# retinal-information-processing-lab/gaussian_processes

Hardware: AMD Instinct MI355X
Metric: GP fits/sec (kernel+chol+solve+grad loglik) at N=8192 d=256 (higher is better)
Workload: dtype f64; 1 GPU; N=8192 d=256 single cell f64, one M-step closure evaluation with 6 gradients (BASELINE configs[2], headline); N=8192, d=256, parallelism=independent units over 1 GPU(s), one process per GPU, no data-path collective

## Files before the change

### gaussian_processes_amd/_lib.py

```python
from __future__ import annotations

import ctypes
import os

from .build import lib_path

vp, i32, i64, f64 = ctypes.c_void_p, ctypes.c_int, ctypes.c_int64, ctypes.c_double
pd = ctypes.POINTER(ctypes.c_double)



class DevGemmArgs(ctypes.Structure):
    _fields_ = ([(n, vp) for n in ("A", "B", "C")] + [(n, i64) for n in ("lda", "ldb", "ldc", "sA", "sB", "sC")] +
                [("alpha", f64), ("beta", f64)] +
                [(n, vp) for n in ("sk_ws", "aux", "sumsq", "Ap", "Bp", "Cp", "auxp", "sumsqp")] +
                [(n, ctypes.c_int32) for n in ("M", "N", "K", "a_kmajor", "b_kmajor", "out_lower", "a_tri", "b_tri", "batch",
                                               "split_k", "tile", "walk", "epi", "nptr", "k_slabs", "b_split")])


class DevGemmRoute(ctypes.Structure):
    _fields_ = [(n, ctypes.c_int32) for n in ("rc", "tile", "sk_first", "xcd", "stages", "half_occ", "edge", "epi",
                                              "sumsq_entries", "blocks", "pair", "slabs")]


_SIGS = {
    "gpfit_version": (i32, []),
    "gpfit_last_error": (ctypes.c_char_p, []),
    "gpfit_dgemm": (i32, [vp, i32, i32, i32, i32, i32, f64, vp, i64, vp, i64, f64, vp, i64, i32, i32, i32]),
    "gpfit_dgemm_ex": (i32, [vp, i32, i32, i32, i32, i32, f64, vp, i64, vp, i64, f64, vp, i64, i32, i32, i32, i32, i32]),
    "gpfit_ctx_create": (i32, [i32, i64, i64, i64, ctypes.POINTER(vp)]),
    "gpfit_ctx_destroy": (None, [vp]),
    "gpfit_check_limits": (i32, [pd, pd, pd]),
    "gpfit_localker_mask": (i32, [pd, i32, i32, vp, ctypes.POINTER(i64)]),
    "gpfit_localker": (i32, [vp, vp, pd, i32, i32, vp, i64, vp, vp]),
    "gpfit_acosker": (i32, [vp, vp, f64, vp, i64, i64, vp, i64, i64, i64, vp, i64, vp, vp, i64, vp]),
    "gpfit_acosker_pullback": (i32, [vp, vp, f64, vp, i64, i64, vp, i64, i64, i64, vp, i64, vp, i64, vp, vp, i64, pd]),
    "gpfit_acosker_diag": (i32, [vp, vp, f64, vp, i64, i64, i64, vp, i64, vp, vp, vp]),
    "gpfit_fit_eval": (i32, [vp, vp, pd, pd, pd, i32, i32, vp, i64, i64, vp, vp, vp, i64, f64, f64, i32, pd,
                             vp, vp, vp]),
    "gpfit_potrf": (i32, [vp, vp, vp, i64, i64, vp, i64, vp, i64, pd, ctypes.POINTER(i32)]),
    "gpfit_potrf_append": (i32, [vp, vp, vp, i64, vp, i64, i64, vp, pd, ctypes.POINTER(i32)]),
    "gpfit_potrf_append_block": (i32, [vp, vp, vp, i64, vp, i64, i64, i64, vp, i64, pd, ctypes.POINTER(i32)]),
    "gpfit_estep": (i32, [vp, vp, vp, i64, i64, vp, vp, vp, f64, vp, vp, i64]),
    "gpfit_estep_projected": (i32, [vp, vp, vp, i64, vp, i64, vp, i64, i64, i64, vp, vp, vp, f64, vp, vp, i64, vp, vp,
                                    vp]),
    "gpfit_estep_projected_damped": (i32, [vp, vp, vp, i64, vp, i64, vp, i64, vp, i64, vp, i64, i64, i64, vp, vp, vp, f64, f64,
                                           vp, vp, i64, ctypes.POINTER(i32)]),
    "gpfit_fparam_eval": (i32, [vp, vp, vp, vp, vp, i64, f64, i32, f64, vp, pd]),
    "gpfit_fparam_lbfgs": (i32, [vp, vp, vp, vp, vp, i64, f64, i32, f64, i32, i32, f64, f64, f64, vp, pd]),
    "gpfit_estep_chain": (i32, [vp, vp, vp, i64, vp, i64, vp, i64, i64, i64, vp, vp, vp, vp, vp, i64, vp, vp, f64, i32, f64,
                                i32, i32, i32, f64, f64, f64, pd]),
    "gpfit_estep_chain_full": (i32, [vp, vp, vp, i64, i64, vp, vp, vp, vp, vp, i64, vp, vp, f64, i32, f64, i32, i32, i32, f64,
                                     f64, f64, pd]),
    "gpfit_estep_chain_batch": (i32, [vp, i32, vp, vp, vp, vp, vp, vp, vp, i64, vp, vp, vp, vp, vp, vp, vp, vp, vp, pd, i32, pd,
                                      i32, i32, i32, f64, f64, f64, pd]),
    "gpfit_estep_chain_full_batch": (i32, [vp, i32, vp, vp, vp, i64, vp, vp, vp, vp, vp, vp, vp, vp, pd, i32, pd, i32, i32, i32,
                                           f64, f64, f64, pd]),
    "gpfit_estep_chain_damped": (i32, [vp, vp, vp, i64, vp, i64, vp, i64, vp, i64, i64, i64, vp, vp, vp, vp, vp, i64, vp, vp,
                                       f64, f64, i32, f64, i32, i32, i32, f64, f64, f64, pd]),
    "gpfit_estep_chain_damped_batch": (i32, [vp, i32, vp, vp, vp, vp, vp, vp, vp, vp, vp, i64, vp, vp, vp, vp, vp, vp, vp, vp,
                                             vp, pd, f64, i32, pd, i32, i32, i32, f64, f64, f64, pd]),
    "gpfit_elbo": (i32, [vp, vp, vp, vp, i64, vp, i64, vp, i64, i64, i32, f64, vp, vp, vp, i64, f64, f64, pd,
                         ctypes.POINTER(i32)]),
    "gpfit_elbo_batch": (i32, [vp, i32, vp, vp, vp, vp, vp, vp, vp, vp, vp, ctypes.POINTER(i32), pd, vp, vp, vp, i64, pd, pd, pd,
                               ctypes.POINTER(i32)]),
    "gpfit_subspace_sweeps": (i32, [vp, vp, vp, i64, i64, i64, vp, vp, vp, vp, i32, pd, i32, ctypes.POINTER(i32)]),
    "gpfit_subspace_sweeps_batch": (i32, [vp, i32, vp, vp, i64, i64, i64, vp, vp, vp, vp, ctypes.POINTER(i32), vp, i32,
                                          ctypes.POINTER(i32)]),
    "gpfit_sign_steps": (i32, [vp, vp, vp, i64, f64, vp, vp, vp, i32, pd, i32, i32, ctypes.POINTER(i32)]),
    "gpfit_sign_steps_batch": (i32, [vp, i32, vp, vp, i64, pd, vp, vp, vp, i32, pd, i32, i32, ctypes.POINTER(i32)]),
    "gpfit_fparam_lbfgs_host": (i32, [vp, vp, vp, i64, f64, i32, f64, i32, i32, f64, f64, f64, vp, pd]),
    "gpfit_set_profile": (i32, [vp, i32]),
    "gpfit_get_profile": (i32, [vp, pd]),
    "gpfit_get_phases": (i32, [vp, pd]),
    "gpfit_last_enqueue_ms": (f64, [vp]),
    "gpfit_fit_eval_f32": (i32, [vp, vp, pd, pd, pd, i32, i32, vp, i64, i64, vp, vp, vp, i64, f64, f64, i32, pd,
                                 vp, vp, vp]),
    "gpfit_fit_eval_finish": (i32, [vp, pd]),
    "gpfit_fit_eval_batch": (i32, [vp, i32, vp, pd, pd, pd, i32, i32, vp, i64, i64, vp, vp, vp, i64, pd, pd, i32, pd,
                                   ctypes.POINTER(i32)]),
    "gpfit_fit_eval_batch_f32": (i32, [vp, i32, vp, pd, pd, pd, i32, i32, vp, i64, i64, vp, vp, vp, i64, pd, pd, i32, pd,
                                       ctypes.POINTER(i32)]),
    "gpfit_fit_eval_projected": (i32, [vp, vp, pd, pd, pd, i32, i32, vp, i64, i64, vp, vp, i64, i64, vp, vp, i64, f64, f64, pd]),
    "gpfit_fit_eval_projected_batch": (i32, [vp, i32, vp, pd, pd, pd, i32, i32, vp, i64, i64, vp, vp, vp, vp, vp, vp, vp, pd, pd,
                                             pd, ctypes.POINTER(i32)]),
    "gpfit_fit_eval_sparse": (i32, [vp, vp, pd, pd, pd, i32, i32, vp, i64, i64, vp, i64, i64, vp, vp, i64, i64, vp, vp, i64,
                                    f64, f64, pd]),
    "gpfit_fit_eval_sparse_batch": (i32, [vp, i32, vp, pd, pd, pd, i32, i32, vp, i64, i64, vp, i64, i64, vp, vp, vp, vp, vp,
                                          vp, vp, pd, pd, pd, ctypes.POINTER(i32)]),
    "gpfit_grad_pullback": (i32, [vp, vp, pd, i32, i32, vp, i64, i64, vp, i64, vp, pd]),
    "gpfit_nd_utility": (i32, [vp, vp, vp, i64, vp, i32, vp]),
    "gpfit_score_pool": (i32, [vp, vp, f64, vp, i64, i64, vp, i64, vp, i64, i64, i64, vp, i64, vp, i64, i64, vp, i64, vp,
                               f64, f64, vp, i32, i64, vp, vp, vp, vp]),
    "gpfit_score_pool_batch": (i32, [vp, i32, vp, pd, vp, vp, i64, vp, vp, vp, vp, vp, vp, vp, vp, vp, vp, vp, vp, vp, vp, pd, pd,
                                     vp, i32, i64, vp, vp, vp, vp]),
    "gpfit_utility_sum": (i32, [vp, vp, i64, i32, vp, i64, vp]),
    "gpfit_probe_mfma_f64": (i32, [vp, vp, i32, i32]),
    "gpfit_probe_stream_copy": (i32, [vp, vp, vp, i64]),
    "gpfit_dev_gemm_route": (i32, [i32, ctypes.POINTER(DevGemmArgs), ctypes.POINTER(DevGemmArgs), ctypes.POINTER(DevGemmRoute)]),
    "gpfit_dev_gemm_plan": (i64, [i32, ctypes.POINTER(DevGemmArgs), i32, ctypes.POINTER(ctypes.c_int32), i64]),
    "gpfit_dev_gemm": (i32, [vp, i32, ctypes.POINTER(DevGemmArgs), ctypes.POINTER(DevGemmArgs)]),
    "gpfit_dev_ctx_copy": (i32, [vp, ctypes.c_char_p, i64, vp, i64, i32]),
    "gpfit_dev_ctx_fill": (i32, [vp, ctypes.c_char_p, i32]),
    "gpfit_dev_potrf": (i32, [vp, vp, i32, i32, vp, vp, vp, vp, vp, i64, i32, ctypes.c_uint32, ctypes.c_uint32, i32]),
}

_lib = None


class GpfitError(RuntimeError):
    pass


def exported_symbols():
    return sorted(_SIGS)


def load():
    global _lib
    if _lib is not None:
        return _lib
    path = lib_path()
    if not os.path.exists(path):
        raise GpfitError(
            f"{path} not found: build it with `python -m gaussian_processes_amd.build` "
            "(there is no CPU fallback for the GP fit path)")
    lib = ctypes.CDLL(path)
    for name, (res, args) in _SIGS.items():
        fn = getattr(lib, name)
        fn.restype = res
        fn.argtypes = args
    _lib = lib
    return lib


def last_error() -> str:
    return load().gpfit_last_error().decode(errors="replace")


def check(rc: int, what: str):
    if rc < 0 and rc != -2:
        raise GpfitError(f"{what} failed (rc={rc}): {last_error()}")
    return rc


def darr(values):
    return (ctypes.c_double * len(values))(*[float(v) for v in values])
```

### gaussian_processes_amd/csrc/api_dev.hip

```cpp
#include "gemm_core.h"
#include "context.h"
#include "gpfit_mi355x.h"

#include <cstring>

namespace gpfit {
namespace {

template <typename R>
int fill(const gpfit_dev_gemm_args& d, GemmArgsT<R>& g) {
  g = GemmArgsT<R>{};
  g.A = (const R*)d.A; g.B = (const R*)d.B; g.C = (R*)d.C;
  g.lda = d.lda; g.ldb = d.ldb; g.ldc = d.ldc;
  g.M = d.M; g.N = d.N; g.K = d.K;
  g.alpha = d.alpha; g.beta = d.beta;
  g.a_kmajor = d.a_kmajor; g.b_kmajor = d.b_kmajor;
  g.out_lower = d.out_lower; g.a_tri = d.a_tri; g.b_tri = d.b_tri;
  g.batch = d.batch > 0 ? d.batch : 1;
  g.sA = d.sA; g.sB = d.sB; g.sC = d.sC;
  g.split_k = d.split_k > 0 ? d.split_k : 1;
  g.k_slabs = d.k_slabs > 0 ? d.k_slabs : 0;
  g.tile = d.tile;
  g.reverse = d.walk & 15;
  g.half_occ = (d.walk >> 4) & 1;
  g.sk_ws = d.sk_ws;
  g.epi = d.epi;
  g.aux = (R*)d.aux;
  g.sumsq = d.sumsq;
  g.b_split = d.b_split;
  g.nptr = d.nptr;
  if (d.nptr < 0 || d.nptr > GEMM_MAXB) return d.nptr < 0 ? -3 : 0;
  for (int b = 0; b < d.nptr; ++b) {
    if (!d.Ap || !d.Bp || !d.Cp) return -3;
    g.Ap[b] = (const R*)d.Ap[b];
    g.Bp[b] = (const R*)d.Bp[b];
    g.Cp[b] = (R*)d.Cp[b];
    g.auxp[b] = d.auxp ? (R*)d.auxp[b] : nullptr;
    g.sumsqp[b] = d.sumsqp ? d.sumsqp[b] : nullptr;
  }
  return 0;
}

template <typename R>
int route(const gpfit_dev_gemm_args& d, const gpfit_dev_gemm_args* d2, gpfit_dev_gemm_route_t& o) {
  std::memset(&o, 0, sizeof(o));
  o.sk_first = -1;
  GemmArgsT<R> a, b;
  if (fill(d, a) != 0 || (d2 && fill(*d2, b) != 0)) return -3;
  GemmRoute r = d2 ? gemm_pair_shape(a, b) : gemm_route(a);
  long blocks = d2 ? r.tiles : -1;
  if (r.rc == 0 && r.sched == GEMM_STREAMK) {
    SkHostPlan plan;
    if (streamk_plan_host(a, r.sk_first, plan) != 0) r.stay_data_parallel();
    else blocks = plan.blocks;
  }
  if (r.rc == 0 && r.sched == GEMM_XCD) {
    std::vector<int> table;
    if (xcd_plan_host(a, table) != 0) return -3;
    r.gx = (int)table.size();
  }
  o.rc = r.rc; o.tile = r.tile; o.sk_first = r.sk_first; o.xcd = r.sched == GEMM_XCD; o.stages = r.stages;
  o.half_occ = r.half; o.edge = r.edge; o.epi = r.epi; o.sumsq_entries = r.sumsq_entries; o.slabs = r.slabs;
  o.pair = d2 && r.rc == 0;
  o.blocks = (int)std::min<long>(blocks >= 0 ? blocks : (long)r.gx * r.gy * r.gz, 0x7fffffffL);
  return 0;
}

template <typename R>
int64_t plan(const gpfit_dev_gemm_args& d, int kind, int32_t* out, int64_t cap) {
  GemmArgsT<R> a;
  if (fill(d, a) != 0 || a.M <= 0 || a.N <= 0) return -3;
  const GemmRoute r = gemm_route(a);
  if (r.rc != 0) return -3;
  if (kind == 1) {
    if (r.sched != GEMM_XCD) return -1;
    std::vector<int> table;
    if (xcd_plan_host(a, table) != 0) return -1;
    const int64_t need = 1 + (int64_t)table.size();
    if (need > cap || !out) return need;
    out[0] = (int32_t)table.size();
    std::memcpy(out + 1, table.data(), table.size() * sizeof(int));
    return need;
  }
  if (kind == 4) {
    if (r.sched != GEMM_XCD) return -1;
    std::vector<int> table;
    if (xcd_plan_host(a, table) != 0) return -1;
    const int64_t need = 1 + 3 * (int64_t)table.size();
    if (need > cap || !out) return need;
    out[0] = (int32_t)table.size();
    for (size_t e = 0; e < table.size(); ++e) {
      const int t = table[e];
      KRange kr{0, 0};
      if (t >= 0) kr = gemm_tile_k_range(a.a_tri, a.b_tri, a.K, (t >> 16) * TILE, (t & 0xffff) * TILE, TILE, a.b_split);
      out[1 + 3 * e] = t; out[2 + 3 * e] = kr.beg; out[3 + 3 * e] = kr.end;
    }
    return need;
  }
  if (kind == 3) {
    if (a.k_slabs <= 0) return -1;
    const SlabPlan sp = slab_plan(a.M, a.k_slabs);
    const int64_t need = 4 + 4 * (int64_t)sp.items;
    if (need > cap || !out) return need;
    out[0] = sp.items; out[1] = sp.live; out[2] = sp.ks * SLAB_TILE; out[3] = SLAB_TILE;
    for (int e = 0; e < sp.items; ++e) {
      int ti, z;
      slab_item(sp, e, ti, z);
      int32_t* w = out + 4 + 4 * e;
      w[0] = ti; w[1] = z;
      const KRange kr = gemm_tile_k_range(a.a_tri, a.b_tri, a.K, ti * SLAB_TILE, 0, SLAB_TILE);
      w[2] = std::max(kr.beg, z * sp.ks * SLAB_TILE);
      w[3] = std::min(kr.end, (z + 1) * sp.ks * SLAB_TILE);
    }
    return need;
  }
  if (kind != 2) return -3;
  if (r.sched != GEMM_STREAMK) return -1;
  const int first = r.sk_first;
  SkHostPlan p;
  if (streamk_plan_host(a, first, p) != 0) return -1;
  const int64_t nt = (int64_t)p.tiles.size(), nfix = (int64_t)p.fix_tile.size(), nslot = (int64_t)p.fix_slot.size();
  const int64_t need = 8 + 5 * nt + nfix + (nfix + 1) + nslot;
  if (need > cap || !out) return need;
  out[0] = first; out[1] = (int32_t)nt; out[2] = p.total; out[3] = p.blocks; out[4] = p.per_block;
  out[5] = (int32_t)nfix; out[6] = (int32_t)nslot;
  out[7] = (int32_t)(SK_WS_BYTES / ((size_t)TILE * TILE * sizeof(double)));
  int32_t* w = out + 8;
  for (const SkTile& t : p.tiles) { *w++ = t.row0; *w++ = t.col0; *w++ = t.kbeg; *w++ = t.ksteps; *w++ = t.prefix; }
  std::memcpy(w, p.fix_tile.data(), nfix * sizeof(int)); w += nfix;
  std::memcpy(w, p.fix_ptr.data(), (nfix + 1) * sizeof(int)); w += nfix + 1;
  std::memcpy(w, p.fix_slot.data(), nslot * sizeof(int));
  return need;
}

template <typename R>
int run(hipStream_t s, const gpfit_dev_gemm_args& d, const gpfit_dev_gemm_args* d2) {
  GemmArgsT<R> a, b;
  if (fill(d, a) != 0 || (d2 && fill(*d2, b) != 0)) {
    set_error("gpfit_dev_gemm: a pointer batch needs its pointer arrays");
    return -3;
  }
  return d2 ? launch_gemm_pair(a, b, gemm_pair_shape(a, b), s) : launch_gemm(a, s);
}

struct CtxBuf { void* p; int64_t bytes; };
CtxBuf ctx_buffer(gpfit_ctx* c, const char* name) {
  const int64_t np = c->np_cap, dp = c->dp_cap, nn = np * np * 8;
  const struct { const char* n; double* p; int64_t bytes; } tab[] = {
      {"Abuf", c->Abuf, nn}, {"Tbuf", c->Tbuf, nn}, {"Wbuf", c->Wbuf, nn}, {"Zbuf", c->Zbuf, nn}, {"Cos", c->Cos, nn},
      {"TmpV", c->TmpV, nn}, {"Xm", c->Xm, np * dp * 8}, {"Xt2", c->Xt2, np * dp * 8}, {"Ybuf", c->Ybuf, np * dp * 8},
      {"Mmat", c->Mmat, dp * dp * 8}, {"Cmat", c->Cmat, dp * dp * 8}, {"tvec", c->tvec, 2 * np * 8}, {"bv", c->bv, np * 8},
      {"q", c->q, np * 8}, {"wl", c->wl, np * 8}, {"q2", c->q2, np * 8}, {"dq1", c->dq1, np * 8}, {"dq2", c->dq2, np * 8}};
  for (const auto& t : tab)
    if (std::strcmp(t.n, name) == 0) return {t.p, t.bytes};
  return {nullptr, 0};
}

template <typename R>
int potrf(gpfit_ctx* c, hipStream_t s, int nb, void* const* A, void* const* L, void* const* Li, void* const* Tmp,
          int* const* info, int64_t ld, int n, uint32_t need, uint32_t halves, int side_min) {
  CholBatchT<R> B;
  B.nb = nb;
  for (int b = 0; b < nb; ++b) {
    B.A[b] = (R*)A[b]; B.L[b] = (R*)L[b]; B.Li[b] = (R*)Li[b]; B.Tmp[b] = (R*)Tmp[b];
    B.info[b] = info[b];
  }
  B.ld = ld;
  if (side_min > 0) {
    GP_TRY(ensure_side_stream(c));
    B.ctx = c; B.side_min = side_min;
    c->side_ev_next = 0;
  }
  return potrf_lockstep<R>(B, 0, n, need, main_lane(c, s), halves);
}

}
}

extern "C" {

int gpfit_dev_gemm_route(int is_f32, const gpfit_dev_gemm_args* args, const gpfit_dev_gemm_args* pair_args,
                         gpfit_dev_gemm_route_t* out) {
  if (!args || !out) return -3;
  return is_f32 ? gpfit::route<float>(*args, pair_args, *out) : gpfit::route<double>(*args, pair_args, *out);
}

int64_t gpfit_dev_gemm_plan(int is_f32, const gpfit_dev_gemm_args* args, int kind, int32_t* out, int64_t cap) {
  if (!args) return -3;
  return is_f32 ? gpfit::plan<float>(*args, kind, out, cap) : gpfit::plan<double>(*args, kind, out, cap);
}

int gpfit_dev_gemm(void* stream, int is_f32, const gpfit_dev_gemm_args* args, const gpfit_dev_gemm_args* pair_args) {
  if (!args) return -3;
  return is_f32 ? gpfit::run<float>((hipStream_t)stream, *args, pair_args)
                : gpfit::run<double>((hipStream_t)stream, *args, pair_args);
}

int gpfit_dev_potrf(gpfit_ctx* ctx, void* stream, int is_f32, int nb, void* const* A, void* const* L, void* const* Li,
                    void* const* Tmp, int* const* info, int64_t ld, int n, uint32_t need, uint32_t halves, int side_min) {
  const int64_t elem = is_f32 ? 4 : 8;
  bool ok = ctx && A && L && Li && Tmp && info && nb >= 1 && nb <= gpfit::GEMM_MAXB && n > 0 && n % gpfit::TILE == 0 &&
            ld >= n && (ld * elem) % 16 == 0 && side_min >= 0;
  if (ok) {
    const uint32_t all = nb >= 32 ? 0xffffffffu : ((1u << nb) - 1u);
    ok = ((need | halves) & ~all) == 0;
    for (int b = 0; b < nb && ok; ++b) ok = A[b] && L[b] && Li[b] && Tmp[b] && info[b];
  }
  if (!ok) {
    gpfit::set_error("gpfit_dev_potrf: bad argument");
    return -3;
  }
  GP_CTX_ENTER(ctx, "gpfit_dev_potrf");
  return is_f32 ? gpfit::potrf<float>(ctx, (hipStream_t)stream, nb, A, L, Li, Tmp, info, ld, n, need, halves, side_min)
                : gpfit::potrf<double>(ctx, (hipStream_t)stream, nb, A, L, Li, Tmp, info, ld, n, need, halves, side_min);
}

int gpfit_dev_ctx_copy(gpfit_ctx* ctx, const char* name, int64_t offset, void* dev, int64_t bytes, int to_ctx) {
  if (!ctx || !name || !dev || offset < 0 || bytes < 0 || ctx->pend.active) return -3;
  gpfit::DeviceGuard guard(ctx->device);
  const gpfit::CtxBuf b = gpfit::ctx_buffer(ctx, name);
  if (!b.p || offset + bytes > b.bytes) return -3;
  GP_HIP(hipDeviceSynchronize());
  char* w = (char*)b.p + offset;
  GP_HIP(hipMemcpy(to_ctx ? (void*)w : dev, to_ctx ? dev : (void*)w, (size_t)bytes, hipMemcpyDeviceToDevice));
  GP_HIP(hipDeviceSynchronize());
  return 0;
}

int gpfit_dev_ctx_fill(gpfit_ctx* ctx, const char* name, int byte) {
  if (!ctx || !name || ctx->pend.active) return -3;
  gpfit::DeviceGuard guard(ctx->device);
  const gpfit::CtxBuf b = gpfit::ctx_buffer(ctx, name);
  if (!b.p) return -3;
  GP_HIP(hipDeviceSynchronize());
  GP_HIP(hipMemset(b.p, byte, (size_t)b.bytes));
  GP_HIP(hipDeviceSynchronize());
  return 0;
}

}
```

### gaussian_processes_amd/csrc/common.h

```cpp
#pragma once
#include <hip/hip_runtime.h>
#include <stdint.h>
#include <stdio.h>
#include <string>

namespace gpfit {

constexpr double PI32 = 3.1415927410125732;

constexpr int TILE = 128;
constexpr int TRMV_ROWS = 128;
constexpr int KTILE = 16;

void set_error(const std::string& msg);

#define GP_HIP(expr)                                                                     \
  do {                                                                                   \
    hipError_t _e = (expr);                                                              \
    if (_e != hipSuccess) {                                                              \
      gpfit::set_error(std::string(#expr) + ": " + hipGetErrorString(_e));               \
      return -100;                                                                       \
    }                                                                                    \
  } while (0)

#define GP_TRY(expr)            \
  do {                          \
    int _rc = (expr);           \
    if (_rc != 0) return _rc;   \
  } while (0)

inline int64_t round_up(int64_t x, int64_t m) { return (x + m - 1) / m * m; }

constexpr int GEMM_MAXB = 32;

template <typename R>
struct GemmArgsT {
  const R* A;
  const R* B;
  R* C;
  int64_t lda, ldb, ldc;
  int M, N, K;
  double alpha, beta;
  int a_kmajor, b_kmajor;
  int out_lower;
  int a_tri, b_tri;
  int batch;
  int64_t sA, sB, sC;
  int split_k;
  int k_slabs;
  int tile;
  int reverse;
  int half_occ;
  void* sk_ws;
  int b_split;
  const int* sched;
  int epi;
  R* aux;
  double* sumsq;
  int nptr;
  const R* Ap[GEMM_MAXB];
  const R* Bp[GEMM_MAXB];
  R* Cp[GEMM_MAXB];
  R* auxp[GEMM_MAXB];
  double* sumsqp[GEMM_MAXB];
  const R* B2;
};
using GemmArgs = GemmArgsT<double>;

constexpr int SLAB_TILE = 64;
struct SlabPlan {
  int nt, ks, live;
  int full, rb;
  int items;
};
__host__ __device__ inline SlabPlan slab_plan(int M, int slabs) {
  SlabPlan p;
  p.nt = (M + SLAB_TILE - 1) / SLAB_TILE;
  p.ks = (p.nt + slabs - 1) / slabs;
  p.live = (p.nt + p.ks - 1) / p.ks;
  p.full = p.live + p.ks * (p.live * (p.live - 1) / 2);
  p.rb = p.nt - (p.live - 1) * p.ks;
  p.items = p.full + (p.rb - 1) * p.live + (p.ks - p.rb) * (p.live - 1);
  return p;
}
__host__ __device__ inline void slab_item(const SlabPlan& p, int e, int& ti, int& z) {
  if (e < p.full) {
    for (z = 0; e >= z * p.ks + 1; ++z) e -= z * p.ks + 1;
    ti = e;
    return;
  }
  e -= p.full;
  int r;
  const int head = (p.rb - 1) * p.live;
  if (e < head) {
    r = 1 + e / p.live;
    z = e % p.live;
  } else {
    e -= head;
    r = p.rb + e / (p.live - 1);
    z = e % (p.live - 1);
  }
  ti = z * p.ks + r;
}

constexpr size_t SK_WS_BYTES = (size_t)2 * 512 * TILE * TILE * sizeof(double);

template <typename R> constexpr int ktile_of() { return 128 / (int)sizeof(R); }

enum { GEMM_DATA_PARALLEL = 0, GEMM_XCD = 1, GEMM_STREAMK = 2 };
struct GemmRoute {
  int rc;
  const char* error;
  int sched;
  int sk_first;
  int tile;
  int tiles, tiles_n;
  int stages;
  int edge;
  int half;
  int gx, gy, gz;
  int epi;
  int sumsq_entries;
  int slabs;
  void stay_data_parallel() { sched = GEMM_DATA_PARALLEL; sk_first = -1; gx = tiles; }
};
template <typename R> GemmRoute gemm_route(const GemmArgsT<R>& a);
template <typename R> int gemm_pick_tile(const GemmArgsT<R>& a);
template <typename R> int launch_gemm(const GemmArgsT<R>& a, const GemmRoute& r, hipStream_t s);
template <typename R> int launch_gemm(const GemmArgsT<R>& a, hipStream_t s) { return launch_gemm(a, gemm_route(a), s); }
template <typename R> int launch_gemm_streamk(const GemmArgsT<R>& a, const GemmRoute& r, hipStream_t s);
template <typename R> int launch_gemm_xcd(const GemmArgsT<R>& a, GemmRoute r, hipStream_t s);
template <typename R> int launch_gemm_plain(const GemmArgsT<R>& a, const GemmRoute& r, hipStream_t s);
template <typename R> GemmRoute gemm_pair_shape(const GemmArgsT<R>& a, const GemmArgsT<R>& b);
template <typename R> int launch_gemm_pair(const GemmArgsT<R>& a, const GemmArgsT<R>& b, const GemmRoute& h, hipStream_t s);

template <typename R>
struct GramArgsT {
  const R* XCt;
  const R* Xt;
  const R* q1;
  const R* q2;
  R* Kout;
  R* Cos;
  int64_t ld1, ld2, ldk;
  int64_t ldcos;
  int np1, np2, nv1, nv2, Kd;
  double s0sq;
  int lower;
  int pad_identity;
  int mirror;
};
using GramArgs = GramArgsT<double>;
template <typename R> int launch_gram(const GramArgsT<R>& a, hipStream_t s);

}
```

### gaussian_processes_amd/csrc/fit.hip

```cpp
#include "units.h"
#include "gemm_core.h"
#include "gpfit_mi355x.h"

#include <algorithm>
#include <chrono>
#include <cmath>
#include <cstdlib>
#include <cstring>
#include <limits>

namespace gpfit {

static thread_local gpfit_ctx* g_prof = nullptr;

static int walk(Walk which) {
  static int w[W_COUNT] = {3, 2, 1, 9, 9, 2, 2};
  static bool init = false;
  if (!init) {
    init = true;
    if (const char* e = getenv("GPFIT_WALKS")) {
      int v[W_COUNT];
      if (sscanf(e, "%d,%d,%d,%d,%d,%d,%d", &v[0], &v[1], &v[2], &v[3], &v[4], &v[5], &v[6]) == 7)
        for (int i = 0; i < W_COUNT; ++i) w[i] = v[i];
    }
  }
  return w[which];
}

static hipEvent_t prof_event(gpfit_ctx* c) {
  hipEvent_t e;
  if (!c->ev_pool.empty()) {
    e = c->ev_pool.back();
    c->ev_pool.pop_back();
    return e;
  }
  (void)hipEventCreate(&e);
  return e;
}

void prof_begin(gpfit_ctx* c) {
  if (c->profile == 1) {
    g_prof = c;
    c->prof.clear();
  }
}

void prof_end(gpfit_ctx* c) {
  if (g_prof != c) return;
  g_prof = nullptr;
  (void)hipDeviceSynchronize();
  double ms[4] = {0, 0, 0, 0}, fl[4] = {0, 0, 0, 0}, cnt[4] = {0, 0, 0, 0};
  double big_ms = 0, big_fl = 0;
  for (auto& r : c->prof) {
    float t = 0.f;
    (void)hipEventElapsedTime(&t, r.a, r.b);
    if (r.kind == 0 && r.flops > big_fl) { big_fl = r.flops; big_ms = t; }
    ms[r.kind] += t;
    fl[r.kind] += r.flops;
    cnt[r.kind] += 1;
    c->ev_pool.push_back(r.a);
    c->ev_pool.push_back(r.b);
  }
  c->prof.clear();
  c->prof_out[0] = ms[0]; c->prof_out[1] = fl[0]; c->prof_out[2] = cnt[0];
  c->prof_out[3] = ms[1]; c->prof_out[4] = cnt[1];
  c->prof_out[5] = ms[2]; c->prof_out[6] = fl[2]; c->prof_out[7] = cnt[2];
  c->prof_out[8] = ms[3]; c->prof_out[9] = fl[3]; c->prof_out[10] = cnt[3];
  c->prof_out[11] = big_ms; c->prof_out[12] = big_fl;
}

ProfScope::ProfScope(hipStream_t s_, double flops_, int kind_) : s(s_), flops(flops_), kind(kind_) {
  if (g_prof) {
    a = prof_event(g_prof);
    (void)hipEventRecord(a, s);
  }
}
ProfScope::~ProfScope() {
  if (g_prof && a) {
    hipEvent_t b = prof_event(g_prof);
    (void)hipEventRecord(b, s);
    g_prof->prof.push_back({a, b, flops, kind});
  }
}

template <typename R>
double gemm_flops(const GemmArgsT<R>& g, int T) {
  const int tm = (g.M + T - 1) / T, tn = (g.N + T - 1) / T, r = TILE / T;
  double steps = 0;
  for (int ti = 0; ti < tm; ++ti)
    for (int tj = 0; tj < tn; ++tj) {
      if (g.out_lower && tj / r > ti / r) continue;
      const KRange kr = gemm_tile_k_range(g.a_tri, g.b_tri, g.K, ti * T, tj * T, T, g.b_split);
      if (kr.end > kr.beg) steps += (kr.end - kr.beg);
    }
  return 2.0 * T * T * steps * (g.nptr > 0 ? g.nptr : (g.batch > 0 ? g.batch : 1));
}

static int g_eval_count = 0;
static int gemm_log_eval() {
  static const int v = getenv("GPFIT_GEMM_LOG") ? atoi(getenv("GPFIT_GEMM_LOG")) : -1;
  return v;
}
static bool gemm_logging() { return gemm_log_eval() >= 0 && g_eval_count == gemm_log_eval(); }
template <typename R>
static void gemm_log_tail(const char* tag, const GemmArgsT<R>& g, const char* end) {
  fprintf(stderr, "%s alpha %g beta %g lda %lld ldb %lld ldc %lld walk %d split %d slabs %d%s", tag, g.alpha, g.beta, (long long)g.lda,
          (long long)g.ldb, (long long)g.ldc, g.reverse, g.split_k, g.k_slabs, end);
}

template <typename R>
int run_gemm(hipStream_t s, const GemmArgsT<R>& g, const GemmRoute& r) {
  if (gemm_logging()) {
    fprintf(stderr, "[gpfit gemm] M %d N %d K %d atri %d btri %d lower %d nb %d tile %d ak %d bk %d epi %d flops %.6e", g.M, g.N, g.K,
            g.a_tri, g.b_tri, g.out_lower, g.nptr > 0 ? g.nptr : 1, r.tile, g.a_kmajor, g.b_kmajor, g.epi, gemm_flops(g, r.tile));
    gemm_log_tail("", g, "");
    if (g.b_split > 0) fprintf(stderr, " bsplit %d", g.b_split);
    fprintf(stderr, "\n");
  }
  ProfScope ps(s, g_prof ? gemm_flops(g, r.tile) : 0.0, (g_prof && r.tile != TILE) ? 3 : 0);
  return launch_gemm(g, r, s);
}
template int run_gemm<double>(hipStream_t, const GemmArgsT<double>&, const GemmRoute&);
template int run_gemm<float>(hipStream_t, const GemmArgsT<float>&, const GemmRoute&);

static int splitk_for(int M, int N, int K) {
  const long tiles = (long)((M + TILE - 1) / TILE) * ((N + TILE - 1) / TILE);
  if (tiles >= 384) return 1;
  long sp = (768 + tiles - 1) / tiles;
  sp = std::min<long>(sp, std::max(1, K / 256));
  return (int)std::max<long>(1, sp);
}
template <typename R>
static int gemm_splitk_list(Lane lane, Dims d, double alpha, const Operand<R>& a, const Operand<R>& b, const Mat<R>& C,
                            R* const* partial, const int64_t* partial_elems) {
  static const bool off = getenv("GPFIT_NO_SPLITK") != nullptr;
  const int64_t slab = (int64_t)d.M * C.ld;
  int splits[GEMM_MAXB];
  bool any = false;
  for (int i = 0; i < C.cnt; ++i) {
    splits[i] = (off || !partial[i]) ? 1 : (int)std::min<int64_t>(splitk_for(d.M, d.N, d.K), partial_elems[i] / std::max<int64_t>(1, slab));
    any = any || splits[i] > 1;
  }
  if (!any) return product(lane, d, alpha, a, b, into(C));
  for (int i = 0; i < C.cnt; ++i) {
    Operand<R> ai = a, bi = b;
    ai.m.cnt = bi.m.cnt = 1;
    ai.m.p[0] = a.m.p[i]; bi.m.p[0] = b.m.p[i];
    if (splits[i] <= 1) {
      GP_TRY(product(lane, d, alpha, ai, bi, into(mat(C.p[i], C.ld))));
      continue;
    }
    GemmArgsT<R> g = product_args(lane, d, alpha, ai, bi, into(mat(partial[i], C.ld)));
    g.split_k = splits[i];
    g.sC = slab;
    g.tile = TILE;
    GP_TRY(run_gemm(lane.s, g));
    GP_TRY(launch_reduce_slices(partial[i], slab, splits[i], C.p[i], slab, lane.s));
  }
  return 0;
}

static int fused_epilogues() {
  static const int v = getenv("GPFIT_FUSED_EPI") ? atoi(getenv("GPFIT_FUSED_EPI")) : 15;
  return v;
}

template <typename R>
int product(Lane lane, Dims d, double alpha, const Operand<R>& a, const Operand<R>& b, const Output<R>& c, int walk, Epilogue<R>* e) {
  const int cnt = c.m.cnt, epi = e ? e->which : 0;
  if (e) { e->carried = false; e->sumsq_entries = 0; }
  if (cnt <= 0) return 0;
  if (cnt > GEMM_MAXB) {
    set_error("product: more problems than a pointer batch holds");
    return -3;
  }
  GemmArgsT<R> g = product_args(lane, d, alpha, a, b, c, walk);
  static const bool no_batch = getenv("GPFIT_NO_BATCH") != nullptr;
  if (cnt == 1 || gemm_pick_tile(g) == TILE || no_batch) {
    auto problem = [&](int i, bool fused) {
      g.A = a.m.p[i]; g.B = b.m.p[i]; g.C = c.m.p[i]; g.B2 = b.split > 0 ? b.p2[i] : nullptr;
      g.epi = fused ? epi : 0; g.aux = fused ? e->aux[i] : nullptr; g.sumsq = fused ? e->sumsq[i] : nullptr;
    };
    GemmRoute routes[GEMM_MAXB];
    bool fused = epi != 0;
    for (int i = 0; i < cnt && fused; ++i) {
      problem(i, true);
      routes[i] = gemm_route(g);
      fused = routes[i].epi != 0;
    }
    for (int i = 0; i < cnt; ++i) {
      problem(i, fused);
      GP_TRY(fused ? run_gemm(lane.s, g, routes[i]) : run_gemm(lane.s, g));
    }
    if (e) e->carried = fused;
    if (fused) e->sumsq_entries = routes[0].sumsq_entries;
    return 0;
  }
  g = batch_args(lane, d, alpha, a, b, c, walk, e);
  GemmRoute r = gemm_route(g);
  if (epi && r.epi == 0) {
    g.epi = 0;
    r = gemm_route(g);
  }
  if (e) { e->carried = g.epi != 0; e->sumsq_entries = r.sumsq_entries; }
  return run_gemm(lane.s, g, r);
}
template int product<double>(Lane, Dims, double, const Operand<double>&, const Operand<double>&, const Output<double>&, int,
                             Epilogue<double>*);
template int product<float>(Lane, Dims, double, const Operand<float>&, const Operand<float>&, const Output<float>&, int,
                            Epilogue<float>*);

constexpr int VSOLVE_MIN = 4096;
static int vsolve_min() {
  static const int v = getenv("GPFIT_VSOLVE_MIN") ? atoi(getenv("GPFIT_VSOLVE_MIN")) : VSOLVE_MIN;
  return v;
}

template <typename R>
int potrf_lockstep(const CholBatchT<R>& B, int r0, int n, uint32_t need, Lane lane, uint32_t halves) {
  const int64_t ld = B.ld;
  const hipStream_t s = lane.s;
  const uint32_t all = (B.nb >= 32) ? 0xffffffffu : ((1u << B.nb) - 1u);
  auto off = [&](int r, int c) { return (int64_t)r * ld + c; };
  auto blk = [&](uint32_t mask, R* const* X, int r, int c) {
    Mat<R> m{};
    m.ld = ld;
    for (int b = 0; b < B.nb; ++b)
      if (mask & (1u << b)) m.p[m.cnt++] = X[b] + off(r, c);
    return m;
  };
  if (n == TILE) {
    ProfScope ps(s, 0.0, 1);
    LeafBatchT<R> bt{};
    bt.n = B.nb;
    for (int b = 0; b < B.nb; ++b) {
      bt.A[b] = B.A[b] + off(r0, r0); bt.L[b] = B.L[b] + off(r0, r0); bt.Li[b] = B.Li[b] + off(r0, r0);
      bt.info[b] = B.info[b];
    }
    bt.lda = bt.ldl = bt.ldi = ld;
    bt.info_base = r0;
    return launch_chol_leaf_batch(bt, s);
  }
  const int k = n / TILE;
  const int n1 = ((k + 1) / 2) * TILE, n2 = n - n1;
  const int r1 = r0 + n1;
  const uint32_t sub = (vsolve_min() > 0 && n1 >= vsolve_min() && n1 >= 2 * TILE) ? (all & ~(need | halves)) : 0u;
  const uint32_t full = all & ~sub;
  GP_TRY(potrf_lockstep<R>(B, r0, n1, full, lane, sub));
  if (full)
    GP_TRY(product(lane, {n2, n1, n1}, 1.0, plain(blk(full, B.A, r1, r0)), trans(tril(blk(full, B.Li, r0, r0))),
                   into(blk(full, B.L, r1, r0)), walk(W_TRSM)));
  if (sub) {
    const int h1 = ((n1 / TILE + 1) / 2) * TILE, h2 = n1 - h1;
    auto half_solve = [&](Dims d, const Operand<R>& y, const Operand<R>& li, const Output<R>& z) -> int {
      const bool one_round = gemm_pick_tile(product_args(lane, d, 1.0, y, li, z, walk(W_TRSM))) == TILE &&
                             (long)(d.M / TILE) * (d.N / TILE) < 2 * SK_SLOTS;
      return product(lane, d, 1.0, y, li, one_round ? on_tiles(z, 64) : z, walk(W_TRSM));
    };
    GP_TRY(half_solve({n2, h1, h1}, plain(blk(sub, B.A, r1, r0)), trans(tril(blk(sub, B.Li, r0, r0))), into(blk(sub, B.L, r1, r0))));
    GP_TRY(product(lane, {n2, h2, h1}, -1.0, plain(blk(sub, B.L, r1, r0)), trans(blk(sub, B.L, r0 + h1, r0)),
                   into(blk(sub, B.A, r1, r0 + h1), 1.0)));
    GP_TRY(half_solve({n2, h2, h2}, plain(blk(sub, B.A, r1, r0 + h1)), trans(tril(blk(sub, B.Li, r0 + h1, r0 + h1))),
                      into(blk(sub, B.L, r1, r0 + h1))));
  }
  const Operand<R> L21 = plain(blk(all, B.L, r1, r0)), L21t = trans(blk(all, B.L, r1, r0));
  const Output<R> A22 = into_lower(blk(all, B.A, r1, r1), 1.0);
  const Operand<R> L21n = plain(blk(need, B.L, r1, r0)), Li11 = plain(tril(blk(need, B.Li, r0, r0)));
  const Output<R> tmp = into(blk(need, B.Tmp, r1, r0));
  const Dims syrk{n2, n2, n1}, merge1{n2, n1, n1};
  hipEvent_t joined = nullptr;
  if (need && B.ctx && B.side_min > 0 && n >= B.side_min && B.ctx->side) {
    gpfit_ctx* c = B.ctx;
    auto next_event = [&]() {
      if (c->side_ev_next == (int)c->side_ev.size()) {
        hipEvent_t e = nullptr;
        (void)hipEventCreateWithFlags(&e, hipEventDisableTiming);
        c->side_ev.push_back(e);
      }
      return c->side_ev[c->side_ev_next++];
    };
    hipEvent_t fork = next_event();
    joined = next_event();
    GP_HIP(hipEventRecord(fork, s));
    GP_HIP(hipStreamWaitEvent(c->side, fork, 0));
    GP_TRY(product(side_lane(c), merge1, 1.0, L21n, Li11, tmp, walk(W_TMP)));
    GP_HIP(hipEventRecord(joined, c->side));
  }
  bool merged = false;
  if (need && !joined) {
    static const bool no_batch = getenv("GPFIT_NO_BATCH") != nullptr;
    const GemmArgsT<R> g2 = batch_args(lane, syrk, -1.0, L21, L21t, A22);
    const GemmArgsT<R> g3 = batch_args(lane, merge1, 1.0, L21n, Li11, tmp, walk(W_TMP));
    const GemmRoute pr = no_batch ? GemmRoute{} : gemm_pair_shape(g2, g3);
    if (!no_batch && pr.rc == 0) {
      if (gemm_logging()) {
        fprintf(stderr, "[gpfit gemm] pair: M %d N %d K %d lower 1 nb %d + M %d N %d K %d btri 1 nb %d tile %d flops %.6e", g2.M, g2.N,
                g2.K, g2.nptr, g3.M, g3.N, g3.K, g3.nptr, pr.tile, gemm_flops(g2, pr.tile) + gemm_flops(g3, pr.tile));
        gemm_log_tail(" a:", g2, "");
        gemm_log_tail(" b:", g3, "\n");
      }
      ProfScope ps(s, g_prof ? gemm_flops(g2, pr.tile) + gemm_flops(g3, pr.tile) : 0.0, 3);
      GP_TRY(launch_gemm_pair(g2, g3, pr, s));
      merged = true;
    }
  }
  if (!merged) GP_TRY(product(lane, syrk, -1.0, L21, L21t, A22));
  GP_TRY(potrf_lockstep<R>(B, r1, n2, need | halves, lane));
  if (need) {
    if (joined) GP_HIP(hipStreamWaitEvent(s, joined, 0));
    else if (!merged) GP_TRY(product(lane, merge1, 1.0, L21n, Li11, tmp, walk(W_TMP)));
    GP_TRY(product(lane, {n2, n1, n2}, -1.0, plain(tril(blk(need, B.Li, r1, r1))), plain(blk(need, B.Tmp, r1, r0)),
                   into(blk(need, B.Li, r1, r0)), walk(W_MERGE)));
  }
  return 0;
}

template int potrf_lockstep<double>(const CholBatchT<double>&, int, int, uint32_t, Lane, uint32_t);
template int potrf_lockstep<float>(const CholBatchT<float>&, int, int, uint32_t, Lane, uint32_t);

template <typename R>
struct TwoSidedBufs { R* Q; const R* Li; R *W, *Z, *H; const R* L; int64_t ld; int min_split; };
template <typename R, typename P>
static Mat<P> ts_blk(int cnt, const TwoSidedBufs<R>* b, const int* r0, P* TwoSidedBufs<R>::*X, int dr, int dc) {
  return mats(cnt, b[0].ld, [&](int i) { const int o = r0 ? r0[i] : 0; return b[i].*X + (int64_t)(o + dr) * b[i].ld + o + dc; });
}
template <typename R>
static int dual_update_list(Lane lane, Dims d, double alpha, const Operand<R>& a, const Operand<R>& b, const Mat<R>& H,
                            const Mat<R>& Z, int wk) {
  const int cnt = H.cnt;
  const int64_t ld = H.ld;
  Epilogue<R> e{4};
  for (int i = 0; i < cnt; ++i) e.aux[i] = Z.p[i];
  bool fused = false;
  if (fused_epilogues() & 4) {
    GemmArgsT<R> g = product_args(lane, d, alpha, a, b, into(H), wk);
    g.epi = 4; g.aux = Z.p[0];
    static const bool no_batch = getenv("GPFIT_NO_BATCH") != nullptr;
    if (cnt > 1 && gemm_pick_tile(g) != TILE && !no_batch) { g.nptr = cnt; g.batch = cnt; }
    fused = gemm_route(g).epi != 0;
  }
  if (fused) {
    GP_TRY(product(lane, d, alpha, a, b, into(H), wk, &e));
    if (!e.carried) {
      set_error("two_sided: the dual-update epilogue was announced but not carried");
      return -100;
    }
    return 0;
  }
  for (int i = 0; i < cnt; ++i)
    GP_HIP(hipMemcpy2DAsync(H.p[i], (size_t)ld * sizeof(R), Z.p[i], (size_t)ld * sizeof(R), (size_t)d.N * sizeof(R), (size_t)d.M,
                            hipMemcpyDeviceToDevice, lane.s));
  GP_TRY(product(lane, d, alpha, a, b, into(H, 1.0), wk));
  for (int i = 0; i < cnt; ++i) GP_TRY(launch_axpby_block<R>(Z.p[i], ld, H.p[i], ld, d.M, d.N, 1.0, 1.0, lane.s));
  return 0;
}

template <typename R>
static int two_sided_list(Lane lane, int cnt, const TwoSidedBufs<R>* b, const int* r0, int n) {
  if (cnt <= 0) return 0;
  using TS = TwoSidedBufs<R>;
  auto blk = [&](auto X, int dr, int dc) { return ts_blk(cnt, b, r0, X, dr, dc); };
  const int k = n / TILE;
  if (n < b[0].min_split || k < 2) {
    static const int wbase_walk = getenv("GPFIT_WBASE_WALK") ? atoi(getenv("GPFIT_WBASE_WALK")) : 0;
    GP_TRY(product(lane, {n, n, n}, 1.0, trans(blk(&TS::Q, 0, 0)), plain(tril(blk(&TS::Li, 0, 0))), into(blk(&TS::Z, 0, 0)),
                   walk(W_RBASE)));
    return product(lane, {n, n, n}, 0.5, trans(tril(blk(&TS::Li, 0, 0))), plain(blk(&TS::Z, 0, 0)),
                   into_lower(blk(&TS::W, 0, 0)), wbase_walk);
  }
  const int n1 = ((k + 1) / 2) * TILE, n2 = n - n1;
  auto diagonal_blocks = [&]() -> int {
    TwoSidedBufs<R> bb[GEMM_MAXB];
    int rr[GEMM_MAXB];
    if (n1 == n2 && 2 * cnt <= GEMM_MAXB) {
      for (int i = 0; i < cnt; ++i) {
        bb[2 * i] = b[i]; rr[2 * i] = r0[i];
        bb[2 * i + 1] = b[i]; rr[2 * i + 1] = r0[i] + n1;
      }
      return two_sided_list<R>(lane, 2 * cnt, bb, rr, n1);
    }
    for (int i = 0; i < cnt; ++i) rr[i] = r0[i] + n1;
    GP_TRY(two_sided_list<R>(lane, cnt, b, r0, n1));
    return two_sided_list<R>(lane, cnt, b, rr, n2);
  };
  GP_TRY(product(lane, {n2, n1, n2}, 0.5, trans(blk(&TS::Q, n1, n1)), plain(blk(&TS::Li, n1, 0)), into(blk(&TS::Z, n1, 0))));
  GP_TRY(dual_update_list(lane, {n2, n1, n1}, 1.0, plain(blk(&TS::Q, n1, 0)), plain(tril(blk(&TS::Li, 0, 0))), blk(&TS::H, n1, 0),
                          blk(&TS::Z, n1, 0), walk(W_H)));
  static const int w21_walk = getenv("GPFIT_W21_WALK") ? atoi(getenv("GPFIT_W21_WALK")) : 0;
  GP_TRY(product(lane, {n2, n1, n2}, 0.5, trans(tril(blk(&TS::Li, n1, n1))), plain(blk(&TS::Z, n1, 0)),
                 into(blk(&TS::W, n1, 0)), w21_walk));
  GP_TRY(diagonal_blocks());
  GP_TRY(product(lane, {n1, n1, n2}, 0.5, trans(blk(&TS::Li, n1, 0)), plain(blk(&TS::H, n1, 0)), into_lower(blk(&TS::W, 0, 0), 1.0)));
  return product(lane, {n1, n1, n2}, 0.5, trans(blk(&TS::H, n1, 0)), plain(blk(&TS::Li, n1, 0)), into_lower(blk(&TS::W, 0, 0), 1.0));
}

constexpr int TOP_BLOCKS_MIN = 2048, TOP_BLOCKS_MIN_F32 = 5120;
static bool top_in_blocks(int np, size_t elem_bytes) { return np >= (elem_bytes == 4 ? TOP_BLOCKS_MIN_F32 : TOP_BLOCKS_MIN); }

template <typename R>
static int two_sided_top(Lane lane, int cnt, const TwoSidedBufs<R>* b, int n) {
  if (cnt <= 0) return 0;
  using TS = TwoSidedBufs<R>;
  const hipStream_t s = lane.s;
  const int64_t ld = b[0].ld;
  auto blk = [&](auto X, int r, int c) { return ts_blk(cnt, b, (const int*)nullptr, X, r, c); };
  int rr[GEMM_MAXB];
  const int k = n / TILE;
  const int n1 = ((k + 1) / 2) * TILE, n2 = n - n1;
  for (int i = 0; i < cnt; ++i) rr[i] = n1;
  GP_TRY(two_sided_list<R>(lane, cnt, b, rr, n2));
  for (int i = 0; i < cnt; ++i) GP_TRY(launch_symmetrize(b[i].W + (int64_t)n1 * ld + n1, ld, n2, s));
  static const int w21_walk = getenv("GPFIT_W21_WALK") ? atoi(getenv("GPFIT_W21_WALK")) : 0;
  GP_TRY(product(lane, {n2, n1, n2}, 0.5, trans(tril(blk(&TS::Li, n1, n1))), plain(blk(&TS::Q, n1, 0)),
                 into(blk(&TS::Z, n1, 0)), w21_walk));
  GP_TRY(dual_update_list(lane, {n2, n1, n2}, -1.0, plain(blk(&TS::W, n1, n1)), plain(blk(&TS::L, n1, 0)), blk(&TS::H, n1, 0),
                          blk(&TS::Z, n1, 0), 0));
  GP_TRY(product(lane, {n2, n1, n1}, 1.0, plain(blk(&TS::H, n1, 0)), plain(tril(blk(&TS::Li, 0, 0))), into(blk(&TS::W, n1, 0)),
                 walk(W_H)));
  GP_TRY(product(lane, {n1, n1, n2}, -1.0, trans(blk(&TS::L, n1, 0)), plain(blk(&TS::Z, n1, 0)), into_lower(blk(&TS::Q, 0, 0), 1.0)));
  GP_TRY(product(lane, {n1, n1, n2}, -1.0, trans(blk(&TS::Z, n1, 0)), plain(blk(&TS::L, n1, 0)), into_lower(blk(&TS::Q, 0, 0), 1.0)));
  for (int i = 0; i < cnt; ++i) GP_TRY(launch_symmetrize(b[i].Q, ld, n1, s));
  for (int i = 0; i < cnt; ++i) rr[i] = 0;
  return two_sided_list<R>(lane, cnt, b, rr, n1);
}

static double lin_pm1_host(int i, int n) {
  if (n <= 1) return -1.0;
  const double step = 2.0 / (double)(n - 1);
  return (i < n / 2) ? std::fma(step, (double)i, -1.0) : std::fma(-step, (double)(n - 1 - i), 1.0);
}

static int compute_mask(const double* theta, int n_rows, int n_cols, uint8_t* mask, int* pix) {
  const double eb = std::exp(theta[3]);
  int d = 0;
  for (int p = 0; p < n_rows * n_cols; ++p) {
    const double x = lin_pm1_host(p % n_cols, n_cols), y = lin_pm1_host(p / n_cols, n_rows);
    const double dx = x - theta[1], dy = y - theta[2];
    const double alpha = std::exp(-eb * (dx * dx + dy * dy));
    const bool keep = alpha >= 0.001;
    if (mask) mask[p] = keep ? 1 : 0;
    if (keep) {
      if (pix) pix[d] = p;
      ++d;
    }
  }
  return d;
}

static Theta make_theta(const double* t) {
  Theta th;
  th.sigma0 = t[0]; th.eps0x = t[1]; th.eps0y = t[2]; th.logbeta = t[3]; th.logrho = t[4]; th.amp = t[5];
  th.eb = std::exp(t[3]);
  th.er = std::exp(t[4]);
  return th;
}

static int check_limits(const double* theta, const double* lower, const double* upper) {
  static const char* names[6] = {"sigma_0", "eps_0x", "eps_0y", "-2log2beta", "-log2rho2", "Amp"};
  for (int i = 0; i < 6; ++i) {
    if (!(lower[i] <= theta[i] && theta[i] <= upper[i])) {
      char buf[256];
      snprintf(buf, sizeof buf, "%s = %.4f is not within the limits of %g and %g", names[i], theta[i], lower[i],
               upper[i]);
      set_error(buf);
      return -2;
    }
  }
  return 0;
}

int ensure_side_stream(gpfit_ctx* c) {
  if (c->side) return 0;
  int least = 0, greatest = 0;
  GP_HIP(hipDeviceGetStreamPriorityRange(&least, &greatest));
  GP_HIP(hipStreamCreateWithPriority(&c->side, hipStreamNonBlocking, least));
  return 0;
}

template <typename T>
static int dev_alloc(gpfit_ctx* c, T** p, size_t count) {
  void* q = nullptr;
  GP_HIP(hipMalloc(&q, count * sizeof(T)));
  c->allocs.push_back(q);
  *p = (T*)q;
  return 0;
}

template <typename R>
static R* ws_as(double* b) { return reinterpret_cast<R*>(b); }

static void fill_out_of_box(double* out) {
  const double inf = std::numeric_limits<double>::infinity();
  out[OUT_LOSS] = inf;
  out[OUT_LOGLIK] = out[OUT_KL] = std::numeric_limits<double>::quiet_NaN();
  for (int i = 0; i < 6; ++i) out[OUT_GRAD + i] = inf;
}

struct Admitted { int d, dp; Theta th; };
static int admit(gpfit_ctx* c, const char* name, const char* whose, const double* theta, const double* lower,
                 const double* upper, int n_rows, int n_cols, int np, double* out, Admitted* a) {
  if (lower && upper && check_limits(theta, lower, upper) != 0) {
    fill_out_of_box(out);
    return -2;
  }
  if (np > c->np_cap || n_rows * n_cols > c->dfull_cap) {
    set_error(std::string(name) + ": problem larger than " + whose + " capacity");
    return -3;
  }
  a->d = compute_mask(theta, n_rows, n_cols, nullptr, c->pix_host);
  a->dp = (int)round_up(a->d, 32);
  if (a->d <= 0 || a->dp > c->dp_cap) {
    set_error(std::string(name) + ": masked pixel count is zero or exceeds " + whose + " capacity");
    return -3;
  }
  a->th = make_theta(theta);
  return 0;
}

template <typename R>
static int build_metric(gpfit_ctx* c, hipStream_t s, const Theta& th, int d, int dp, int n_rows, int n_cols) {
  return launch_localker<R>(th, c->pix, d, dp, n_rows, n_cols, ws_as<R>(c->Cmat), dp, nullptr, s);
}
template <typename R>
static int kernel_side(gpfit_ctx* c, Lane lane, const R* X, int64_t ldx, int n, int np, int d, int dp, double s0sq,
                       R* Xt, R* XCt, R* Xm, R* Kvec, R* q) {
  const int64_t ld = np;
  const hipStream_t s = lane.s;
  GP_TRY(launch_gather(X, ldx, n, c->pix, d, dp, np, Xt, ld, Xm, dp, s));
  GP_TRY(product(lane, {dp, np, dp}, 1.0, trans(mat(ws_as<R>(c->Cmat), dp)), plain(mat(Xt, ld)), into(mat(XCt, ld))));
  return launch_qvec(Xt, XCt, ld, dp, n, np, s0sq, Kvec, q, s);
}
template <typename R>
static int gram_square(hipStream_t s, const R* XCt, const R* Xt, const R* q, R* Kout, R* Cos, int n, int np, int dp,
                       double s0sq, int mirror) {
  GramArgsT<R> g{};
  g.XCt = XCt; g.Xt = Xt; g.q1 = q; g.q2 = q; g.Kout = Kout; g.Cos = Cos;
  g.ld1 = np; g.ld2 = np; g.ldk = np; g.np1 = np; g.np2 = np; g.nv1 = n; g.nv2 = n; g.Kd = dp;
  g.s0sq = s0sq; g.lower = 1; g.pad_identity = 1;
  g.mirror = mirror;
  ProfScope ps(s, (double)np * (np + TILE) * dp, 2);
  return launch_gram(g, s);
}
template <typename R>
static int build_kernel(gpfit_ctx* c, Lane lane, const Theta& th, int d, int dp, int n_rows, int n_cols, const R* X,
                        int64_t ldx, int n, int np, int mirror) {
  const double s0sq = th.sigma0 * th.sigma0;
  const hipStream_t s = lane.s;
  GP_TRY(build_metric<R>(c, s, th, d, dp, n_rows, n_cols));
  GP_TRY(kernel_side<R>(c, lane, X, ldx, n, np, d, dp, s0sq, ws_as<R>(c->Xt), ws_as<R>(c->XCt), ws_as<R>(c->Xm),
                        ws_as<R>(c->Kvec), ws_as<R>(c->q)));
  return gram_square<R>(s, ws_as<R>(c->XCt), ws_as<R>(c->Xt), ws_as<R>(c->q), ws_as<R>(c->Kbuf), ws_as<R>(c->Cos), n, np,
                        dp, s0sq, mirror);
}

template <typename R>
static int solve_mean(gpfit_ctx* c, int np, bool blocks, hipStream_t s) {
  const int64_t ld = np;
  R *m = ws_as<R>(c->mpad), *y = ws_as<R>(c->yv), *b = ws_as<R>(c->bv);
  if (!blocks) {
    GP_TRY(launch_trmv_lower(ws_as<R>(c->Libuf), ld, np, m, y, s));
    GP_TRY(launch_dot(y, y, np, c->scal + S_MKM, s));
    return launch_trmv_lower_t(ws_as<R>(c->Libuf), ld, np, y, b, c->trmv_part, s);
  }
  const int kt = np / TILE, n1 = ((kt + 1) / 2) * TILE, n2 = np - n1;
  const R *A = ws_as<R>(c->Libuf), *C = A + (int64_t)n1 * ld + n1, *L21 = ws_as<R>(c->Lbuf) + (int64_t)n1 * ld;
  GP_TRY(launch_trmv_lower(A, ld, n1, m, y, s));
  GP_TRY(launch_gemv_sub(L21, ld, n2, n1, y, m + n1, b + n1, s));
  GP_TRY(launch_trmv_lower(C, ld, n2, b + n1, y + n1, s));
  GP_TRY(launch_dot(y, y, np, c->scal + S_MKM, s));
  GP_TRY(launch_trmv_lower_t(C, ld, n2, y + n1, b + n1, c->trmv_part, s));
  GP_TRY(launch_gemv_t_sub(L21, ld, n2, n1, b + n1, y, b, c->trmv_part, s));
  return launch_trmv_lower_t(A, ld, n1, b, b, c->trmv_part, s);
}

template <typename R>
static int adjoint_pass(gpfit_ctx* c, hipStream_t s, const R* W, const R* Cos, const R* bv, const R* q, const R* wl, int n,
                        int np, R* A, R* tvec) {
  GP_TRY(launch_adjoint(W, Cos, (int64_t)np, bv, q, n, np, A, c->upart, c->vpart, c->sumA_part, s));
  const int t64 = np / 64;
  return launch_adjoint_reduce(c->upart, c->vpart, c->sumA_part, t64, t64 * (t64 + 1) / 2, q, wl, n, np, tvec, c->rpad,
                               c->scal + S_ADJ, s);
}
template <typename R>
static int xty(gpfit_ctx* c, hipStream_t s, const R* Xa, const R* Yb, int np, int dp, R* out, bool prof, bool sym = false) {
  GemmArgsT<R> g = product_args(Lane{s, nullptr}, {dp, dp, np}, 1.0, trans(mat(Xa, dp)), plain(mat(Yb, dp)),
                                into(mat(ws_as<R>(c->Mpart), dp)));
  g.split_k = c->split_k_M; g.sC = (int64_t)dp * dp;
  const GemmRoute r = gemm_route(g);
  if (prof) {
    ProfScope ps(s, g_prof ? gemm_flops(g, r.tile) : 0.0, (g_prof && r.tile != TILE) ? 3 : 0);
    GP_TRY(launch_gemm(g, r, s));
  } else {
    GP_TRY(launch_gemm(g, r, s));
  }
  if (sym) return launch_reduce_slices_sym(ws_as<R>(c->Mpart), (int64_t)dp * dp, c->split_k_M, out, dp, s);
  return launch_reduce_slices(ws_as<R>(c->Mpart), (int64_t)dp * dp, c->split_k_M, out, (int64_t)dp * dp, s);
}
static int pullback_slabs(int np, int dp) {
  const int nt = np / SLAB_TILE;
  return std::max(1, std::min(nt >= 32 ? 4 : (nt >= 8 ? 2 : 1), np / dp));
}
template <typename R>
static int lambda_t_x_list(Lane lane, const Operand<R>& a, const Operand<R>& b, const Mat<R>& Y, const Mat<R>& scratch, int np, int dp) {
  const int cnt = Y.cnt;
  if (cnt <= 0 || cnt > GEMM_MAXB) return cnt == 0 ? 0 : -3;
  const int slabs = pullback_slabs(np, dp);
  const SlabPlan sp = slab_plan(np, slabs);
  const bool direct = sp.live == 1;
  const Output<R> c = into(direct ? Y : scratch);
  GemmArgsT<R> g = cnt > 1 ? batch_args(lane, {np, dp, np}, 1.0, a, b, c) : product_args(lane, {np, dp, np}, 1.0, a, b, c);
  g.k_slabs = slabs;
  g.sC = (int64_t)np * dp;
  GP_TRY(run_gemm(lane.s, g));
  if (direct) return 0;
  for (int i = 0; i < cnt; ++i)
    GP_TRY(launch_reduce_slabs(scratch.p[i], (int64_t)np * dp, sp.live, sp.ks * SLAB_TILE, Y.p[i], np, dp, lane.s));
  return 0;
}
static int pullback_to_metric(gpfit_ctx* c, Lane lane, const double* W, const double* Cos, const double* q, int n,
                              int np, int dp, double* A, const double* Xm, double* scratch) {
  const hipStream_t s = lane.s;
  GP_TRY(adjoint_pass<double>(c, s, W, Cos, c->bv, q, c->wl, n, np, A, c->tvec));
  GP_TRY(lambda_t_x_list(lane, trans(tril(mat(A, np))), plain(mat(Xm, dp)), mat(c->Ybuf, dp), mat(scratch, dp), np, dp));
  GP_TRY(launch_rowscale_add(c->Ybuf, dp, Xm, dp, c->tvec, np, dp, s, 0.5));
  return xty<double>(c, s, Xm, c->Ybuf, np, dp, c->Mmat, false, true);
}

struct ProjChain { double *Va, *Vl, *Vli, *Vt; };
static int projected_factor(Lane lane, const Units& U, const double* const* V_b, const int64_t* ldvb, const int* nk, int nb,
                            const ProjChain* vc) {
  if (U.cnt == 0) return 0;
  const int cnt = U.cnt;
  const int64_t lb = nb;
  const hipStream_t s = lane.s;
  CholBatchT<double> cb;
  uint32_t kchains = 0;
  for (int i = 0; i < cnt; ++i) {
    const ProjChain& v = vc[U.at[i]];
    kchains |= 1u << add_v_chain(cb, U.ctx[i], INFO_K);
    add_chain(cb, v.Va, v.Vl, v.Vli, v.Vt, U.ctx[i]->info + INFO_V);
  }
  cb.ld = lb; cb.ctx = nullptr; cb.side_min = 0;
  GP_TRY(potrf_lockstep<double>(cb, 0, nb, kchains, lane));
  const PerUnit<int> nks = U.from(nk);
  GP_TRY(launch_logdet_pair_group(cnt, U.table<const double*>([&](int u) { return vc[u].Vl; }), U.scal(S_LOGDET_V),
                                  U.cof(&gpfit_ctx::LVbuf), U.scal(S_LOGDET_K), lb, nks, s));
  GP_TRY(product(lane, {nb, nb, nb}, 1.0, trans(tril(U.mats(&gpfit_ctx::LiVbuf, lb))), plain(tril(U.mats(&gpfit_ctx::LiVbuf, lb))),
                 into_lower(U.mats(&gpfit_ctx::Vbuf, lb))));
  GP_TRY(launch_symmetrize_group(cnt, U.of(&gpfit_ctx::Vbuf), lb, nb, s));
  GP_TRY(launch_pack_lower_group(cnt, U.from(V_b), U.from(ldvb), nks, U.of(&gpfit_ctx::LVbuf), lb, nb, s));
  return launch_symmetrize_group(cnt, U.of(&gpfit_ctx::LVbuf), lb, nb, s);
}
static int projected_kl_products(Lane lane, const Units& U, const int* nk, int nb) {
  if (U.cnt == 0) return 0;
  const int64_t lb = nb;
  const Mat<double> Ki = U.mats(&gpfit_ctx::Vbuf, lb), S2 = U.mats(&gpfit_ctx::LVbuf, lb), S3 = U.mats(&gpfit_ctx::LiVbuf, lb),
                    S4 = U.mats(&gpfit_ctx::TmpV, lb);
  GP_TRY(product(lane, {nb, nb, nb}, 1.0, plain(Ki), plain(S2), into(S3)));
  GP_TRY(launch_proj_trace_group(U.cnt, U.of(&gpfit_ctx::LiVbuf), lb, U.from(nk), U.scal(S_TRACE), lane.s));
  return product(lane, {nb, nb, nb}, 1.0, plain(S3), plain(Ki), into(S4));
}
static int projected_adjoints(Lane lane, const ProjGroupT& pg, double* const* part, const int64_t* part_elems) {
  auto all = [&](const PerUnit<double*>& X) { return mats(pg.n_units, pg.ld, [&](int i) { return X[i]; }); };
  GP_TRY(launch_symv_lower_group(pg.n_units, pg.Ki, pg.ld, pg.nb, pg.mb, pg.bvec, lane.s));
  GP_TRY(launch_dot_group(pg.n_units, pg.mb, pg.bvec, pg.nb, pg.mkm, lane.s));
  GP_TRY(launch_proj_moments_group(pg, lane.s));
  GP_TRY(launch_proj_ga_group(pg, lane.s));
  GP_TRY(product(lane, {pg.np, pg.nb, pg.nb}, 1.0, plain(all(pg.Ga)), plain(all(pg.Ki)), into(all(pg.GaKi))));
  GP_TRY(gemm_splitk_list(lane, {pg.nb, pg.nb, pg.np}, 1.0, trans(all(pg.am)), plain(all(pg.GaKi)), all(pg.P2), part, part_elems));
  GP_TRY(launch_proj_gktb_group(pg, lane.s));
  return launch_proj_gkb_group(pg, lane.s);
}
static int closure_prepare(const Units& U, const int* d, const int* nk, const double* const* m_b, int nb, hipStream_t s) {
  ClosurePrepT gp{};
  gp.n_units = U.cnt; gp.nb = nb;
  for (int i = 0; i < U.cnt; ++i) {
    gp.pix_host.v[i] = U.ctx[i]->pix_host; gp.cap.v[i] = U.ctx[i]->np_cap; gp.cap_max = std::max(gp.cap_max, U.ctx[i]->np_cap);
  }
  gp.pix = U.of(&gpfit_ctx::pix); gp.info = U.of(&gpfit_ctx::info); gp.d = U.from(d); gp.nk = U.from(nk);
  gp.m_b = U.from(m_b); gp.mpad = U.of(&gpfit_ctx::mpad); gp.bv = U.of(&gpfit_ctx::bv); gp.wl = U.of(&gpfit_ctx::wl);
  return launch_closure_prepare(gp, s);
}
static int closure_collect(const Units& U, hipStream_t s) {
  GroupCollectT gc{};
  gc.n_units = U.cnt;
  for (int i = 0; i < U.cnt; ++i) {
    gpfit_ctx* c = U.ctx[i];
    gc.scal[i] = c->scal; gc.info[i] = c->info; gc.scal_host[i] = c->scal_host; gc.info_host[i] = c->info_host;
  }
  return launch_group_collect(gc, s);
}

static double sigma0_row_metric(const double* sc, double sigma0) { return sigma0 * (2.0 * sc[S_ADJ_SUMA] + 2.0 * sc[S_ADJ]); }
static void grad_rows(const double* sc, double sigma0_row, double* g6) {
  g6[0] = sigma0_row;
  g6[1] = sc[S_D_EPSX];
  g6[2] = sc[S_D_EPSY];
  g6[3] = sc[S_D_BETA];
  g6[4] = sc[S_D_RHO];
  g6[5] = sc[S_D_AMP];
}
static int assemble_out(gpfit_ctx* c, double A, double lambda0, double sigma0_row, int pad, int d, int want_grad,
                        const char* err_K, const char* err_V, double* out_host) {
  const double* sc = c->scal_host;
  const double loglik = A * sc[S_RLAM] + lambda0 * sc[S_SUMR] - sc[S_SUMF];
  const double trKinvV = sc[S_TRACE] - (double)pad;
  const double logdetV = sc[S_LOGDET_V];
  const double KL = -0.5 * logdetV + 0.5 * sc[S_LOGDET_K] + 0.5 * sc[S_MKM] + 0.5 * trKinvV;
  out_host[OUT_LOSS] = -(loglik - KL);
  out_host[OUT_LOGLIK] = loglik;
  out_host[OUT_KL] = KL;
  if (want_grad) grad_rows(sc, sigma0_row, out_host + OUT_GRAD);
  else
    for (int i = 0; i < 6; ++i) out_host[OUT_GRAD + i] = 0.0;
  out_host[OUT_LOGDET_K] = sc[S_LOGDET_K];
  out_host[OUT_LOGDET_V] = logdetV;
  out_host[OUT_TRACE] = trKinvV;
  out_host[OUT_MKM] = sc[S_MKM];
  out_host[OUT_D] = (double)d;
  out_host[OUT_INFO_K] = (double)c->info_host[INFO_K];
  out_host[OUT_INFO_V] = (double)c->info_host[INFO_V];
  if (c->info_host[INFO_K] != 0) {
    set_error(err_K);
    return c->info_host[INFO_K];
  }
  if (c->info_host[INFO_V] != 0) {
// ... 1029 lines not shown
```

### gaussian_processes_amd/csrc/gemm.hip

```cpp
#include "gemm_core.h"

#include <algorithm>
#include <cstdlib>
#include <mutex>
#include <set>
#include <utility>

namespace gpfit {

template <typename R, bool A_KMAJOR, bool B_KMAJOR, bool EDGE, int T, int NS>
__device__ __forceinline__ bool gemm_tile_compute(const GemmArgsT<R>& p, int tiles_n, int ntiles, R* smem,
                                                  typename Real<R>::acc_t (&acc)[T / 32][T / 32], int& ti, int& tj,
                                                  int& row0, int& col0, R*& C) {
  constexpr int KT = Real<R>::KT;

  int slab = 0, slab_tiles = 0;
  const bool slabbed = (T == SLAB_TILE) && p.k_slabs > 0;
  if (slabbed) {
    const SlabPlan sp = slab_plan(p.M, p.k_slabs);
    slab_item(sp, (int)blockIdx.x / tiles_n, ti, slab);
    tj = (int)blockIdx.x % tiles_n;
    slab_tiles = sp.ks;
  } else if (p.sched != nullptr) {
    const int e = p.sched[blockIdx.x];
    if (e < 0) return false;
    ti = e >> 16;
    tj = e & 0xffff;
  } else {
    gemm_walk_tile((int)blockIdx.x, p.reverse, p.out_lower != 0, TILE / T, tiles_n, ntiles, ti, tj);
  }
  row0 = ti * T;
  col0 = tj * T;
  const int b = blockIdx.y, z = blockIdx.z;
  const R* A;
  const R* B;
  if (p.nptr > 0) {
    A = p.Ap[b];
    B = p.Bp[b];
    C = p.Cp[b];
  } else {
    A = p.A + (int64_t)b * p.sA;
    B = p.B + (int64_t)b * p.sB;
    C = p.C + (int64_t)b * p.sC;
  }

  if (p.b_split > 0 && col0 >= p.b_split && p.B2 != nullptr) B = p.B2;
  const KRange kr = gemm_tile_k_range(p.a_tri, p.b_tri, p.K, row0, col0, T, p.b_split);
  int kbeg = kr.beg, kend = kr.end;
  if (slabbed) {
    kbeg = max(kbeg, slab * slab_tiles * T);
    kend = min(kend, (slab + 1) * slab_tiles * T);
    C += (int64_t)slab * p.sC;
  } else if (p.split_k > 1) {
    const int steps = max(0, kend - kbeg) / KT;
    const int per = (steps + p.split_k - 1) / p.split_k;
    const int s0 = min(steps, z * per), s1 = min(steps, (z + 1) * per);
    kend = kbeg + s1 * KT;
    kbeg = kbeg + s0 * KT;
    C += (int64_t)z * p.sC;
  }

#pragma unroll
  for (int i = 0; i < T / 32; ++i)
#pragma unroll
    for (int j = 0; j < T / 32; ++j) acc[i][j] = acc_zero<R>();

  gemm_mainloop<R, A_KMAJOR, B_KMAJOR, EDGE, T, 0, NS>(A, p.lda, B, p.ldb, p.M, p.N, row0, col0, kbeg, kend, smem, acc,
                                                       (p.reverse & 4) != 0);
  return true;
}

template <typename R, bool A_KMAJOR, bool B_KMAJOR, bool EDGE, int T, int NS, int EPI = 0>
__device__ __forceinline__ void gemm_tile_body(const GemmArgsT<R>& p, int tiles_n, int ntiles, R* smem) {
  typename Real<R>::acc_t acc[T / 32][T / 32];
  int ti, tj, row0, col0;
  R* C;
  if (!gemm_tile_compute<R, A_KMAJOR, B_KMAJOR, EDGE, T, NS>(p, tiles_n, ntiles, smem, acc, ti, tj, row0, col0, C)) return;

  const R alpha = (R)p.alpha, beta = (p.split_k > 1 || (T == SLAB_TILE && p.k_slabs > 0)) ? (R)0 : (R)p.beta;
  const int64_t ldc = p.ldc;
  const int M = p.M, N = p.N;
  if constexpr (EPI != 0) {
    constexpr int epi = EPI;
    R* __restrict__ D = p.nptr > 0 ? p.auxp[blockIdx.y] : p.aux;
    double* __restrict__ sumsq = p.nptr > 0 ? p.sumsqp[blockIdx.y] : p.sumsq;
    double ss = 0.0;
    for_each_acc<R, T>(acc, row0, col0, [&](int row, int col, R v) {
      if (EDGE && !(row < M && col < N)) return;
      R o = alpha * v;
      R* c = C + (int64_t)row * ldc + col;
      if (epi & 4) {
        R* dd = D + (int64_t)row * ldc + col;
        const R d0 = *dd;
        o += d0;
        *dd = o + d0;
      } else if (epi & 8) {
        o += D[(int64_t)row * ldc + col];
      } else if (beta != (R)0) {
        o += beta * (*c);
      }
      if (epi & 1) {
        if (row >= col) *c = o;
        if (row > col) C[(int64_t)col * ldc + row] = o;
      } else {
        *c = o;
      }
      if (epi & 2) ss += (double)o * (double)o;
    });
    if (epi & 2) {
#pragma unroll
      for (int o = 32; o > 0; o >>= 1) ss += __shfl_down(ss, o);
      double* red = reinterpret_cast<double*>(smem);
      __syncthreads();
      if ((threadIdx.x & 63) == 0) red[threadIdx.x >> 6] = ss;
      __syncthreads();
      if (threadIdx.x == 0)
        sumsq[p.out_lower ? (int64_t)ti * (ti + 1) / 2 + tj : (int64_t)ti * tiles_n + tj] = (red[0] + red[1]) + (red[2] + red[3]);
    }
    return;
  }
  if (beta == (R)0) {
    for_each_acc<R, T>(acc, row0, col0, [&](int row, int col, R v) {
      if (!EDGE || (row < M && col < N)) C[(int64_t)row * ldc + col] = alpha * v;
    });
  } else {
    for_each_acc<R, T>(acc, row0, col0, [&](int row, int col, R v) {
      if (!EDGE || (row < M && col < N)) {
        R* c = C + (int64_t)row * ldc + col;
        *c = alpha * v + beta * (*c);
      }
    });
  }
}

template <typename R, bool A_KMAJOR, bool B_KMAJOR, bool EDGE, int T, int NS = 2>
__global__ __launch_bounds__(GEMM_THREADS, (T == 128 || NS > 2 ? 2 : 4)) void gemm_mfma_kernel(GemmArgsT<R> p,
                                                                                               int tiles_n,
                                                                                               int ntiles) {
  __shared__ __attribute__((aligned(16))) R smem[2 * NS * Real<R>::KT * T];
  gemm_tile_body<R, A_KMAJOR, B_KMAJOR, EDGE, T, NS>(p, tiles_n, ntiles, smem);
}

#ifdef GPFIT_CLOCK_STAMPS
__device__ long long g_gemm_clock[2][4096][2];
#endif

template <typename R, bool A_KMAJOR, bool B_KMAJOR>
__global__ __launch_bounds__(GEMM_THREADS, 2) void gemm_xcd_kernel(GemmArgsT<R> p, int tiles_n, int ntiles) {
  __shared__ __attribute__((aligned(16))) R smem[4 * Real<R>::KT * TILE];
#ifdef GPFIT_CLOCK_STAMPS
  const long long t0 = __builtin_amdgcn_s_memtime(), w0 = __builtin_amdgcn_s_memrealtime();
#endif
  gemm_tile_body<R, A_KMAJOR, B_KMAJOR, false, TILE, 2>(p, tiles_n, ntiles, smem);
#ifdef GPFIT_CLOCK_STAMPS
  if (threadIdx.x == 0 && blockIdx.x < 4096) {
    g_gemm_clock[B_KMAJOR ? 1 : 0][blockIdx.x][0] = (long long)__builtin_amdgcn_s_memtime() - t0;
    g_gemm_clock[B_KMAJOR ? 1 : 0][blockIdx.x][1] = (long long)__builtin_amdgcn_s_memrealtime() - w0;
  }
#endif
}

template <typename R, bool A_KMAJOR, bool B_KMAJOR, int EPI>
__global__ __launch_bounds__(GEMM_THREADS, 2) void gemm_epi_kernel(GemmArgsT<R> p, int tiles_n, int ntiles) {
  __shared__ __attribute__((aligned(16))) R smem[4 * Real<R>::KT * TILE];
#ifdef GPFIT_CLOCK_STAMPS
  const long long t0 = __builtin_amdgcn_s_memtime(), w0 = __builtin_amdgcn_s_memrealtime();
#endif
  gemm_tile_body<R, A_KMAJOR, B_KMAJOR, false, TILE, 2, EPI>(p, tiles_n, ntiles, smem);
#ifdef GPFIT_CLOCK_STAMPS
  if (threadIdx.x == 0 && blockIdx.x < 4096 && EPI != 4) {
    g_gemm_clock[B_KMAJOR ? 1 : 0][blockIdx.x][0] = (long long)__builtin_amdgcn_s_memtime() - t0;
    g_gemm_clock[B_KMAJOR ? 1 : 0][blockIdx.x][1] = (long long)__builtin_amdgcn_s_memrealtime() - w0;
  }
#endif
}

template <typename R>
int gemm_pick_tile(const GemmArgsT<R>& a) {
  if (a.k_slabs > 0) return SLAB_TILE;
  if (a.tile == 128 || a.tile == 64 || a.tile == 32) return a.tile;
  auto ntiles = [&](int T) {
    const long tm = (a.M + T - 1) / T, tn = (a.N + T - 1) / T;
    const long nb = (a.M + TILE - 1) / TILE;
    return (a.out_lower ? (long)lower_tile_count((int)nb, TILE / T) : tm * tn) * (a.nptr > 0 ? a.nptr : (a.batch > 0 ? a.batch : 1)) *
           (a.split_k > 1 ? a.split_k : 1);
  };
  static const long t128_min = getenv("GPFIT_T128_MIN") ? atol(getenv("GPFIT_T128_MIN")) : 384;
  static const long t128_tri_min = getenv("GPFIT_T128_TRI_MIN") ? atol(getenv("GPFIT_T128_TRI_MIN")) : 1024;
  const bool batch_tri = a.nptr > 0 && (a.a_tri || a.b_tri);
  if (ntiles(128) >= (batch_tri ? t128_tri_min : t128_min)) return 128;
  static const long t64_min = getenv("GPFIT_T64_MIN") ? atol(getenv("GPFIT_T64_MIN")) : 256;
  static const long t32_dim = getenv("GPFIT_T32_DIM") ? atol(getenv("GPFIT_T32_DIM")) : 1024;
  if (ntiles(64) >= t64_min) return 64;
  return (a.M <= t32_dim && a.N <= t32_dim) ? 32 : 64;
}

constexpr int HALF_OCC_LDS = 17 * 1024;
static void allow_dynamic_lds(const void* fn) {
  static std::mutex mu;
  static std::set<std::pair<const void*, int>> done;
  int device = 0;
  (void)hipGetDevice(&device);
  std::lock_guard<std::mutex> lock(mu);
  if (done.insert({fn, device}).second)
    (void)hipFuncSetAttribute(fn, hipFuncAttributeMaxDynamicSharedMemorySize, HALF_OCC_LDS);
}

static int gemm_stages(int T, bool edge, long blocks) {
  static const int deep_max = getenv("GPFIT_DEEP_MAX") ? atoi(getenv("GPFIT_DEEP_MAX")) : 512;
  return (T == TILE || edge || blocks > deep_max) ? 2 : (T == 64 ? 4 : 8);
}

template <typename R>
static int streamk_first_tile(const GemmArgsT<R>& a, long ntiles) {
  static const bool disabled = getenv("GPFIT_NO_STREAMK") != nullptr;
  if (disabled) return -1;
  static const int sk_min = getenv("GPFIT_SK_MIN_TILES") ? atoi(getenv("GPFIT_SK_MIN_TILES")) : 384;
  if (ntiles < sk_min || (long)a.K < 1024) return -1;
  static const int sk_classes = getenv("GPFIT_SK_CLASSES") ? atoi(getenv("GPFIT_SK_CLASSES")) : 5;
  const bool cls1 = (a.a_tri != 0 && a.b_tri != 0), cls2 = (a.out_lower && a.a_tri == 2 && a.b_tri == 0);
  if ((cls1 && !(sk_classes & 1)) || (cls2 && !(sk_classes & 2))) return -1;
  if (cls1 || cls2) return 0;
  if (!(sk_classes & 4)) return -1;
  if (a.a_tri || a.b_tri) return -1;
  const int tail = (int)(ntiles % SK_SLOTS);
  if (tail == 0 || tail >= 384 || ntiles < SK_SLOTS) return -1;
  return (int)ntiles - tail;
}

template <typename R>
GemmRoute gemm_route(const GemmArgsT<R>& a) {
  GemmRoute r{};
  r.sk_first = -1;
  if (a.M <= 0 || a.N <= 0) return r;
  const int T = r.tile = gemm_pick_tile(a);
  auto refuse = [T](const char* why) {
    GemmRoute e{};
    e.rc = -3; e.error = why; e.tile = T; e.sk_first = -1;
    return e;
  };
  const bool strided = a.batch > 1 && a.nptr <= 0;
  r.tiles_n = (a.N + T - 1) / T;
  r.tiles = a.out_lower ? lower_tile_count((a.M + TILE - 1) / TILE, TILE / T) : ((a.M + T - 1) / T) * r.tiles_n;
  r.edge = (a.M % T) || (a.N % T) || (a.out_lower && (a.M % TILE));

  if (T == TILE && !r.edge && a.nptr <= 0 && a.batch <= 1 && a.split_k <= 1 && !a.half_occ &&
      (a.tile == 0 || a.tile == TILE)) {
    static const long xcd_min = getenv("GPFIT_XCD_MIN_TILES") ? atol(getenv("GPFIT_XCD_MIN_TILES")) : 1536;
    const long tm = a.M / TILE, tn = a.N / TILE;
    long ntiles = a.out_lower ? tm * (tm + 1) / 2 : tm * tn;
    if (a.b_split > 0) {
      ntiles = 0;
      for (long ti = 0; ti < tm; ++ti)
        for (long tj = 0; tj < tn; ++tj) {
          const KRange kr = gemm_tile_k_range(a.a_tri, a.b_tri, a.K, (int)ti * TILE, (int)tj * TILE, TILE, a.b_split);
          ntiles += kr.end > kr.beg;
        }
    }
    if ((a.reverse & 8) && !(a.out_lower && a.M != a.N) && tm < 32768 && tn < 32768 && ntiles >= xcd_min) r.sched = GEMM_XCD;
    else if (a.b_split <= 0 && (r.sk_first = streamk_first_tile(a, ntiles)) >= 0) r.sched = GEMM_STREAMK;
  }
  if (a.b_split != 0 && (r.sched != GEMM_XCD || a.b_split < 0 || a.b_split >= a.N || (a.b_split % TILE) || a.b_tri != 1 || a.out_lower))
    return refuse("launch_gemm: a split op(B) needs a lower triangle from a 128-column on and the XCD-aware table (gemm_route says so beforehand)");

  if (a.epi) {
    bool ok = a.split_k <= 1 && a.k_slabs <= 0 && !strided && T == TILE && !(a.M % T) && !(a.N % T) && !a.a_kmajor && !a.half_occ;
    if ((a.epi & 1) && (!a.out_lower || a.M != a.N)) ok = false;
    if ((a.epi & 12) && a.nptr <= 0 && a.aux == nullptr) ok = false;
    if (!((a.epi == 2 && a.b_kmajor) || (a.epi == 1 && !a.b_kmajor) || ((a.epi == 4 || a.epi == 8) && a.b_kmajor))) ok = false;
    if (r.sched == GEMM_STREAMK && !(r.sk_first == 0 && a.out_lower && a.M == a.N && a.epi == 2 && a.sumsq != nullptr)) ok = false;
    if (!ok) return refuse("launch_gemm: this launch cannot carry a fused epilogue (gemm_route says so beforehand)");
  }
  constexpr int EPC = 16 / (int)sizeof(R);
  if (a.K % ktile_of<R>() != 0 || (a.lda % EPC) || (a.ldb % EPC))
    return refuse("launch_gemm: K must be a multiple of the K step and lda, ldb multiples of 16 bytes");
  if (a.out_lower && a.M != a.N) return refuse("launch_gemm: out_lower needs a square output");
  if (a.nptr > 0 && (a.nptr > GEMM_MAXB || a.sched || a.split_k > 1))
    return refuse("launch_gemm: a pointer batch holds at most GEMM_MAXB plain problems");
  if (a.k_slabs > 0 &&
      (a.a_tri != 2 || a.b_tri || a.out_lower || a.M != a.K || (a.M % SLAB_TILE) || a.split_k > 1 || a.sched ||
       a.half_occ || strided || (a.tile != 0 && a.tile != SLAB_TILE)))
    return refuse("launch_gemm: k_slabs needs an upper triangular square op(A) on whole 64-tiles and a plain launch");

  r.epi = a.epi;
  if (a.epi & 2) r.sumsq_entries = (r.sched == GEMM_STREAMK ? 33 : 1) * r.tiles;
  r.gx = r.sched == GEMM_XCD ? 0 : (r.sched == GEMM_STREAMK ? r.sk_first : r.tiles);
  if (a.k_slabs > 0) {
    const SlabPlan sp = slab_plan(a.M, a.k_slabs);
    r.gx = sp.items * r.tiles_n;
    r.slabs = sp.live;
  }
  r.gy = a.nptr > 0 ? a.nptr : std::max(a.batch, 1);
  r.gz = a.split_k > 1 ? a.split_k : 1;
  r.stages = gemm_stages(T, r.edge, (long)r.gx * r.gy * r.gz);
  r.half = T == TILE && a.half_occ;
  return r;
}
template GemmRoute gemm_route<double>(const GemmArgsT<double>&);
template GemmRoute gemm_route<float>(const GemmArgsT<float>&);

template <typename R, int T>
static void launch_T(const GemmArgsT<R>& p, const GemmRoute& r, hipStream_t s) {
  const int tn = r.tiles_n, tiles = r.tiles;
  const bool edge = r.edge, deep = r.stages > 2, half = r.half;
  dim3 grid(r.gx, r.gy, r.gz);
  dim3 block(GEMM_THREADS);
  constexpr int DEEP = (T == 128) ? 2 : (T == 64 ? 4 : 8);
#define GP_LAUNCH(AK, BK, ED)                                                                          \
  do {                                                                                                 \
    if (deep) hipLaunchKernelGGL((gemm_mfma_kernel<R, AK, BK, ED, T, (ED ? 2 : DEEP)>), grid, block, 0, s, p, tn, tiles); \
    else if (half) {                                                                                   \
      allow_dynamic_lds(reinterpret_cast<const void*>(gemm_mfma_kernel<R, AK, BK, ED, T, 2>));          \
      hipLaunchKernelGGL((gemm_mfma_kernel<R, AK, BK, ED, T, 2>), grid, block, HALF_OCC_LDS, s, p, tn, tiles); \
    } else hipLaunchKernelGGL((gemm_mfma_kernel<R, AK, BK, ED, T, 2>), grid, block, 0, s, p, tn, tiles); \
  } while (0)
  if (r.epi) {
    if constexpr (T == TILE) {
      const int key = r.epi * 4 + (p.a_kmajor ? 2 : 0) + (p.b_kmajor ? 1 : 0);
      if (key == 2 * 4 + 1) hipLaunchKernelGGL((gemm_epi_kernel<R, false, true, 2>), grid, block, 0, s, p, tn, tiles);
      else if (key == 1 * 4 + 0) hipLaunchKernelGGL((gemm_epi_kernel<R, false, false, 1>), grid, block, 0, s, p, tn, tiles);
      else if (key == 4 * 4 + 1) hipLaunchKernelGGL((gemm_epi_kernel<R, false, true, 4>), grid, block, 0, s, p, tn, tiles);
      else if (key == 8 * 4 + 1) hipLaunchKernelGGL((gemm_epi_kernel<R, false, true, 8>), grid, block, 0, s, p, tn, tiles);
    }
    return;
  }
  if (p.sched && T == TILE && !edge) {
    switch ((p.a_kmajor ? 2 : 0) | (p.b_kmajor ? 1 : 0)) {
      case 0: hipLaunchKernelGGL((gemm_xcd_kernel<R, false, false>), grid, block, 0, s, p, tn, tiles); break;
      case 1: hipLaunchKernelGGL((gemm_xcd_kernel<R, false, true>), grid, block, 0, s, p, tn, tiles); break;
      case 2: hipLaunchKernelGGL((gemm_xcd_kernel<R, true, false>), grid, block, 0, s, p, tn, tiles); break;
      default: hipLaunchKernelGGL((gemm_xcd_kernel<R, true, true>), grid, block, 0, s, p, tn, tiles); break;
    }
    return;
  }
  const int sel = (p.a_kmajor ? 4 : 0) | (p.b_kmajor ? 2 : 0) | (edge ? 1 : 0);
  switch (sel) {
    case 0: GP_LAUNCH(false, false, false); break;
    case 1: GP_LAUNCH(false, false, true); break;
    case 2: GP_LAUNCH(false, true, false); break;
    case 3: GP_LAUNCH(false, true, true); break;
    case 4: GP_LAUNCH(true, false, false); break;
    case 5: GP_LAUNCH(true, false, true); break;
    case 6: GP_LAUNCH(true, true, false); break;
    case 7: GP_LAUNCH(true, true, true); break;
  }
#undef GP_LAUNCH
}

template <typename R>
int launch_gemm(const GemmArgsT<R>& a, const GemmRoute& route, hipStream_t s) {
  if (route.rc != 0) {
    set_error(route.error);
    return route.rc;
  }
  if (route.tile == 0) return 0;
  if (route.sched == GEMM_XCD) return launch_gemm_xcd(a, route, s);
  if (route.sched != GEMM_STREAMK) return launch_gemm_plain(a, route, s);
  const int rc = launch_gemm_streamk(a, route, s);
  if (rc <= 0) return rc;
  GemmRoute r = route;
  r.stay_data_parallel();
  return launch_gemm_plain(a, r, s);
}

template <typename R>
int launch_gemm_plain(const GemmArgsT<R>& a, const GemmRoute& r, hipStream_t s) {
  GemmArgsT<R> p = a;
  p.batch = r.gy;
  switch (r.tile) {
    case 128: launch_T<R, 128>(p, r, s); break;
    case 64: launch_T<R, 64>(p, r, s); break;
    default: launch_T<R, 32>(p, r, s); break;
  }
  GP_HIP(hipGetLastError());
  return 0;
}

template <typename R>
struct GemmPairT {
  GemmArgsT<R> g[2];
  int tiles[2], tiles_n[2];
};

template <typename R, int T, int NS>
__global__ __launch_bounds__(GEMM_THREADS, (NS > 2 ? 2 : 4)) void gemm_pair_kernel(GemmPairT<R> q) {
  __shared__ __attribute__((aligned(16))) R smem[2 * NS * Real<R>::KT * T];
  const int w = blockIdx.z;
  const GemmArgsT<R>& p = q.g[w];
  if ((int)blockIdx.x >= q.tiles[w] || (int)blockIdx.y >= p.batch) return;
  if (p.b_kmajor) gemm_tile_body<R, false, true, false, T, NS>(p, q.tiles_n[w], q.tiles[w], smem);
  else gemm_tile_body<R, false, false, false, T, NS>(p, q.tiles_n[w], q.tiles[w], smem);
}

template <typename R>
static GemmRoute pair_member_route(const GemmArgsT<R>& a) {
  const GemmRoute none{};
  if (a.nptr <= 0 || a.epi || a.k_slabs > 0 || a.half_occ || a.a_kmajor || (a.M % 64) || (a.N % 64)) return none;
  const GemmRoute r = gemm_route(a);
  return (r.rc == 0 && !r.edge && (r.tile == 32 || r.tile == 64)) ? r : none;
}

template <typename R>
GemmRoute gemm_pair_shape(const GemmArgsT<R>& a, const GemmArgsT<R>& b) {
  static const bool off = getenv("GPFIT_NO_PAIR") != nullptr;
  static const bool no64 = getenv("GPFIT_NO_PAIR64") != nullptr;
  GemmRoute h{};
  h.sk_first = -1;
  const GemmRoute ra = pair_member_route(a), rb = pair_member_route(b);
  if (off || ra.tile == 0 || ra.tile != rb.tile || (no64 && ra.tile == 64)) {
    h.rc = -3;
    h.error = "launch_gemm_pair: the two problems cannot share a launch (gemm_pair_shape says so beforehand)";
    return h;
  }
  h.tile = ra.tile;
  h.tiles = ra.tiles * ra.gy + rb.tiles * rb.gy;
  h.stages = gemm_stages(h.tile, false, h.tiles);
  h.gx = std::max(ra.tiles, rb.tiles);
  h.gy = std::max(ra.gy, rb.gy);
  h.gz = 2;
  return h;
}
template GemmRoute gemm_pair_shape<double>(const GemmArgsT<double>&, const GemmArgsT<double>&);
template GemmRoute gemm_pair_shape<float>(const GemmArgsT<float>&, const GemmArgsT<float>&);

template <typename R>
int launch_gemm_pair(const GemmArgsT<R>& a, const GemmArgsT<R>& b, const GemmRoute& h, hipStream_t s) {
  if (h.rc != 0) {
    set_error(h.error);
    return h.rc;
  }
  static_assert(sizeof(GemmPairT<R>) <= 4096, "kernel arguments are limited to 4 KiB");
  const int T = h.tile;
  GemmPairT<R> q;
  for (int w = 0; w < 2; ++w) {
    q.g[w] = w == 0 ? a : b;
    GemmArgsT<R>& p = q.g[w];
    p.batch = p.nptr;
    q.tiles_n[w] = p.N / T;
    q.tiles[w] = p.out_lower ? lower_tile_count(p.M / TILE, TILE / T) : (p.M / T) * (p.N / T);
  }
  const dim3 grid(h.gx, h.gy, h.gz), block(GEMM_THREADS);
  const bool deep = h.stages > 2;
  if (T == 32 && deep) hipLaunchKernelGGL((gemm_pair_kernel<R, 32, 8>), grid, block, 0, s, q);
  else if (T == 32) hipLaunchKernelGGL((gemm_pair_kernel<R, 32, 2>), grid, block, 0, s, q);
  else if (deep) hipLaunchKernelGGL((gemm_pair_kernel<R, 64, 4>), grid, block, 0, s, q);
  else hipLaunchKernelGGL((gemm_pair_kernel<R, 64, 2>), grid, block, 0, s, q);
  GP_HIP(hipGetLastError());
  return 0;
}
template int launch_gemm_pair<double>(const GemmArgsT<double>&, const GemmArgsT<double>&, const GemmRoute&, hipStream_t);
template int launch_gemm_pair<float>(const GemmArgsT<float>&, const GemmArgsT<float>&, const GemmRoute&, hipStream_t);

template int launch_gemm<double>(const GemmArgsT<double>&, const GemmRoute&, hipStream_t);
template int launch_gemm<float>(const GemmArgsT<float>&, const GemmRoute&, hipStream_t);
template int launch_gemm_plain<double>(const GemmArgsT<double>&, const GemmRoute&, hipStream_t);
template int launch_gemm_plain<float>(const GemmArgsT<float>&, const GemmRoute&, hipStream_t);
template int gemm_pick_tile<double>(const GemmArgsT<double>&);
template int gemm_pick_tile<float>(const GemmArgsT<float>&);

}

#ifdef GPFIT_CLOCK_STAMPS
extern "C" int gpfit_dev_gemm_clock(long long* host_out ) {
  return hipMemcpyFromSymbol(host_out, HIP_SYMBOL(gpfit::g_gemm_clock), sizeof(long long) * 2 * 4096 * 2) == hipSuccess ? 0 : -1;
}
#endif
```

### gaussian_processes_amd/csrc/gemm_sched.hip

```cpp
#include "gemm_core.h"

#include <algorithm>
#include <cstdlib>
#include <map>
#include <mutex>
#include <tuple>
#include <vector>

namespace gpfit {

namespace {
struct Plan {
  int* table = nullptr;
  int blocks = 0;
};
using Key = std::tuple<int, int, int, int, int, int, int, int, int>;
std::map<Key, Plan> g_plans;
std::mutex g_mutex;

struct Item {
  long weight;
  std::vector<int> tiles;
};
}

template <typename R>
int xcd_plan_host(const GemmArgsT<R>& a, std::vector<int>& table) {
  constexpr int KT = 128 / (int)sizeof(R);
  const int tm = a.M / TILE, tn = a.N / TILE;
  auto ksteps = [&](int ti, int tj) {
    const KRange kr = gemm_tile_k_range(a.a_tri, a.b_tri, a.K, ti * TILE, tj * TILE, TILE, a.b_split);
    const int kb = kr.beg, ke = kr.end;
    return std::max(0, ke - kb) / KT;
  };
  const bool skip_empty = a.b_split > 0;
  static const int gr_env = getenv("GPFIT_XCD_GR") ? atoi(getenv("GPFIT_XCD_GR")) : 2;
  static const int gc_env = getenv("GPFIT_XCD_GC") ? atoi(getenv("GPFIT_XCD_GC")) : 2;
  static const int cutdiv = getenv("GPFIT_XCD_CUT") ? atoi(getenv("GPFIT_XCD_CUT")) : 8;
  const int GR = std::max(1, std::min(gr_env, 32)), GC = std::max(1, std::min(gc_env, 32));
  auto make_items = [&](int I0, int I1, int J0, int J1, std::vector<Item>& out) {
    Item it;
    it.weight = 0;
    for (int ti = I0; ti < std::min(I1, tm); ++ti)
      for (int tj = J0; tj < std::min(J1, tn); ++tj) {
        if (a.out_lower && tj > ti) continue;
        if (skip_empty && ksteps(ti, tj) == 0) continue;
        it.tiles.push_back((ti << 16) | tj);
        it.weight += ksteps(ti, tj) + 2;
      }
    if (!it.tiles.empty()) out.push_back(std::move(it));
  };
  std::vector<Item> items;
  for (int I = 0; I < tm; I += GR)
    for (int J = 0; J < tn; J += GC) {
      if (a.out_lower && J >= I + GR) continue;
      make_items(I, I + GR, J, J + GC, items);
    }
  long total = 0;
  for (auto& it : items) total += it.weight;
  const long cut = cutdiv > 0 ? total / 8 / cutdiv : 0;
  std::vector<Item> fine;
  for (auto& it : items) {
    if (it.weight > cut || GR < 2 || GC < 2) { fine.push_back(std::move(it)); continue; }
    const int ti0 = (it.tiles.front() >> 16) / GR * GR, tj0 = (it.tiles.front() & 0xffff) / GC * GC;
    const int hr = (GR + 1) / 2, hc = (GC + 1) / 2;
    make_items(ti0, ti0 + hr, tj0, tj0 + hc, fine);
    make_items(ti0, ti0 + hr, tj0 + hc, tj0 + GC, fine);
    make_items(ti0 + hr, ti0 + GR, tj0, tj0 + hc, fine);
    make_items(ti0 + hr, ti0 + GR, tj0 + hc, tj0 + GC, fine);
  }
  std::stable_sort(fine.begin(), fine.end(), [](const Item& x, const Item& y) { return x.weight > y.weight; });
  std::vector<int> queue[8];
  long load[8] = {0, 0, 0, 0, 0, 0, 0, 0};
  for (auto& it : fine) {
    int best = 0;
    for (int x = 1; x < 8; ++x)
      if (load[x] < load[best]) best = x;
    load[best] += it.weight;
    queue[best].insert(queue[best].end(), it.tiles.begin(), it.tiles.end());
  }
  size_t len = 0;
  for (auto& q : queue) len = std::max(len, q.size());
  table.assign(8 * len, -1);
  for (int x = 0; x < 8; ++x)
    for (size_t i = 0; i < queue[x].size(); ++i) table[8 * i + x] = queue[x][i];
  return 0;
}
template int xcd_plan_host<double>(const GemmArgsT<double>&, std::vector<int>&);
template int xcd_plan_host<float>(const GemmArgsT<float>&, std::vector<int>&);

template <typename R>
static int build(const GemmArgsT<R>& a, Plan& plan) {
  std::vector<int> table;
  GP_TRY(xcd_plan_host(a, table));
  plan.blocks = (int)table.size();
  GP_HIP(hipMalloc((void**)&plan.table, table.size() * sizeof(int)));
  GP_HIP(hipMemcpy(plan.table, table.data(), table.size() * sizeof(int), hipMemcpyHostToDevice));
  return 0;
}

template <typename R>
int launch_gemm_xcd(const GemmArgsT<R>& a, GemmRoute r, hipStream_t s) {
  int device = 0;
  GP_HIP(hipGetDevice(&device));
  Plan plan;
  {
    std::lock_guard<std::mutex> lock(g_mutex);
    const Key key{device, a.M, a.N, a.K, a.out_lower, a.a_tri, a.b_tri, (int)sizeof(R), a.b_split};
    auto it = g_plans.find(key);
    if (it == g_plans.end()) {
      Plan np;
      const int rc = build(a, np);
      if (rc != 0) return rc;
      it = g_plans.emplace(key, np).first;
    }
    plan = it->second;
  }
  GemmArgsT<R> p = a;
  p.sched = plan.table;
  r.gx = plan.blocks;
  p.reverse &= 4;
  return launch_gemm_plain(p, r, s);
}

template int launch_gemm_xcd<double>(const GemmArgsT<double>&, GemmRoute, hipStream_t);
template int launch_gemm_xcd<float>(const GemmArgsT<float>&, GemmRoute, hipStream_t);

}
```

### gaussian_processes_amd/csrc/product.h

```cpp
#pragma once
#include "context.h"
#include <type_traits>

namespace gpfit {

enum Tri { Dense = 0, Lower = 1, Upper = 2 };
struct Dims { int M, N, K; };

template <typename R> struct Mat { int cnt; int64_t ld; Tri tri; R* p[GEMM_MAXB]; };
template <typename R>
Mat<R> mat(R* p, int64_t ld) {
  Mat<R> m{};
  m.cnt = 1; m.ld = ld; m.p[0] = p;
  return m;
}
template <typename F>
auto mats(int cnt, int64_t ld, F&& at) {
  Mat<std::remove_pointer_t<decltype(at(0))>> m{};
  m.cnt = cnt; m.ld = ld;
  for (int i = 0; i < cnt && i < GEMM_MAXB; ++i) m.p[i] = at(i);
  return m;
}
template <typename R> Mat<R> tril(Mat<R> m) { m.tri = Lower; return m; }
template <typename R> Mat<R> triu(Mat<R> m) { m.tri = Upper; return m; }

template <typename R> struct Operand { Mat<const R> m; bool t; int split = 0; const R* p2[GEMM_MAXB] = {}; };
template <typename R> Operand<R> plain(const Mat<const R>& m) { return {m, false}; }
template <typename R> Operand<R> trans(const Mat<const R>& m) { return {m, true}; }
template <typename R> Operand<R> plain(const Mat<R>& m) {
  Operand<R> o{{m.cnt, m.ld, m.tri, {}}, false};
  for (int i = 0; i < m.cnt && i < GEMM_MAXB; ++i) o.m.p[i] = m.p[i];
  return o;
}
template <typename R> Operand<R> trans(const Mat<R>& m) { Operand<R> o = plain(m); o.t = true; return o; }
template <typename R> Operand<R> dense_then_lower(const Mat<R>& dense, const Mat<const R>& lower, int col) {
  Operand<R> o = plain(tril(dense));
  o.split = col;
  for (int i = 0; i < lower.cnt && i < GEMM_MAXB; ++i) o.p2[i] = lower.p[i];
  return o;
}

template <typename R> struct Output { Mat<R> m; bool lower; double beta; int tile = 0; };
template <typename R> Output<R> into(const Mat<R>& m, double beta = 0.0) { return {m, false, beta}; }
template <typename R> Output<R> into_lower(const Mat<R>& m, double beta = 0.0) { return {m, true, beta}; }
template <typename R> Output<R> on_tiles(Output<R> o, int tile) { o.tile = tile; return o; }

template <typename R> struct Epilogue { int which; R* aux[GEMM_MAXB]; double* sumsq[GEMM_MAXB]; bool carried; int sumsq_entries; };

template <typename R>
GemmArgsT<R> product_args(Lane lane, Dims d, double alpha, const Operand<R>& a, const Operand<R>& b, const Output<R>& c,
                          int walk = 0) {
  auto tri = [](const Operand<R>& o) { return (o.t && o.m.tri != Dense) ? (int)Lower + (int)Upper - (int)o.m.tri : (int)o.m.tri; };
  GemmArgsT<R> g{};
  g.A = a.m.p[0]; g.B = b.m.p[0]; g.C = c.m.p[0];
  g.lda = a.m.ld; g.ldb = b.m.ld; g.ldc = c.m.ld;
  g.M = d.M; g.N = d.N; g.K = d.K;
  g.alpha = alpha; g.beta = c.beta;
  g.a_kmajor = a.t ? 1 : 0; g.b_kmajor = b.t ? 0 : 1;
  g.out_lower = c.lower ? 1 : 0; g.a_tri = tri(a); g.b_tri = tri(b);
  g.batch = 1; g.split_k = 1; g.reverse = walk; g.sk_ws = lane.sk_ws;
  g.b_split = b.split; g.B2 = b.split > 0 ? b.p2[0] : nullptr;
  g.tile = c.tile;
  return g;
}
template <typename R>
GemmArgsT<R> batch_args(Lane lane, Dims d, double alpha, const Operand<R>& a, const Operand<R>& b, const Output<R>& c,
                        int walk = 0, const Epilogue<R>* e = nullptr) {
  GemmArgsT<R> g = product_args(lane, d, alpha, a, b, c, walk);
  g.nptr = g.batch = c.m.cnt;
  for (int i = 0; i < c.m.cnt; ++i) {
    g.Ap[i] = a.m.p[i]; g.Bp[i] = b.m.p[i]; g.Cp[i] = c.m.p[i];
    g.auxp[i] = e ? e->aux[i] : nullptr; g.sumsqp[i] = e ? e->sumsq[i] : nullptr;
  }
  g.epi = e ? e->which : 0;
  return g;
}

template <typename R> int run_gemm(hipStream_t s, const GemmArgsT<R>& g, const GemmRoute& r);
template <typename R> int run_gemm(hipStream_t s, const GemmArgsT<R>& g) { return run_gemm(s, g, gemm_route(g)); }
template <typename R>
int product(Lane lane, Dims d, double alpha, const Operand<R>& a, const Operand<R>& b, const Output<R>& c, int walk = 0,
            Epilogue<R>* e = nullptr);

}
```

### include/gpfit_mi355x.h

```cpp
#ifndef GPFIT_MI355X_H
#define GPFIT_MI355X_H

#include <stdint.h>

#ifdef __cplusplus
extern "C" {
#endif

#define GPFIT_VERSION 100

int gpfit_version(void);
const char* gpfit_last_error(void);

int gpfit_dgemm(void* stream, int a_kmajor, int b_kmajor, int M, int N, int K, double alpha,
                const double* A, int64_t lda, const double* B, int64_t ldb, double beta, double* C,
                int64_t ldc, int out_lower, int a_tri, int b_tri);
int gpfit_dgemm_ex(void* stream, int a_kmajor, int b_kmajor, int M, int N, int K, double alpha,
                   const double* A, int64_t lda, const double* B, int64_t ldb, double beta, double* C,
                   int64_t ldc, int out_lower, int a_tri, int b_tri, int walk, int tile);

typedef struct gpfit_ctx gpfit_ctx;
int gpfit_ctx_create(int device, int64_t n_max, int64_t d_max, int64_t d_full_max, gpfit_ctx** out);
void gpfit_ctx_destroy(gpfit_ctx* ctx);

int gpfit_check_limits(const double* theta, const double* lower, const double* upper);

int gpfit_localker_mask(const double* theta, int n_rows, int n_cols, uint8_t* mask_host, int64_t* d_out);

int gpfit_localker(gpfit_ctx* ctx, void* stream, const double* theta, int n_rows, int n_cols,
                   const uint8_t* mask_host, int64_t d, double* C, double* dC);

int gpfit_acosker(gpfit_ctx* ctx, void* stream, double sigma0, const double* x1, int64_t ld1, int64_t n1,
                  const double* x2, int64_t ld2, int64_t n2, int64_t d, const double* C, int64_t ldC,
                  const double* dC, double* K, int64_t ldk, double* dK);

int gpfit_acosker_pullback(gpfit_ctx* ctx, void* stream, double sigma0, const double* x1, int64_t ld1,
                           int64_t n1, const double* x2, int64_t ld2, int64_t n2, int64_t d, const double* C,
                           int64_t ldC, const double* W, int64_t ldw, const double* t1_extra, double* M_out,
                           int64_t ldm, double* out_host);

int gpfit_acosker_diag(gpfit_ctx* ctx, void* stream, double sigma0, const double* x1, int64_t ld1,
                       int64_t n1, int64_t d, const double* C, int64_t ldC, const double* dC, double* Kvec,
                       double* dKvec);

int gpfit_fit_eval(gpfit_ctx* ctx, void* stream, const double* theta, const double* lower,
                   const double* upper, int n_rows, int n_cols, const double* X, int64_t ldx, int64_t N,
                   const double* r, const double* m, const double* V, int64_t ldv, double logA,
                   double lambda0, int want_grad, double* out_host, double* lam_m, double* lam_var,
                   double* f);

int gpfit_fit_eval_finish(gpfit_ctx* ctx, double* out_host);

int gpfit_fit_eval_batch(gpfit_ctx* const* ctxs, int n_units, void* stream, const double* theta,
                         const double* lower, const double* upper, int n_rows, int n_cols,
                         const double* const* X, int64_t ldx, int64_t N, const double* const* r,
                         const double* const* m, const double* const* V, int64_t ldv, const double* logA,
                         const double* lambda0, int want_grad, double* out_host, int* rc_out);
int gpfit_fit_eval_batch_f32(gpfit_ctx* const* ctxs, int n_units, void* stream, const double* theta,
                             const double* lower, const double* upper, int n_rows, int n_cols,
                             const float* const* X, int64_t ldx, int64_t N, const float* const* r,
                             const float* const* m, const float* const* V, int64_t ldv, const double* logA,
                             const double* lambda0, int want_grad, double* out_host, int* rc_out);

int gpfit_grad_pullback(gpfit_ctx* ctx, void* stream, const double* theta, int n_rows, int n_cols,
                        const double* X, int64_t ldx, int64_t N, const double* W, int64_t ldw,
                        const double* gvec, double* out_host);

int gpfit_fit_eval_projected(gpfit_ctx* ctx, void* stream, const double* theta, const double* lower,
                             const double* upper, int n_rows, int n_cols, const double* X, int64_t ldx, int64_t N,
                             const double* r, const double* B, int64_t ldb, int64_t n_kept, const double* m_b,
                             const double* V_b, int64_t ldvb, double logA, double lambda0, double* out_host);

#define GPFIT_FIT_EVAL_PROJECTED_MAX_UNITS 16
int gpfit_fit_eval_projected_batch(gpfit_ctx* const* ctxs, int n_units, void* stream, const double* theta,
                                   const double* lower, const double* upper, int n_rows, int n_cols,
                                   const double* const* X, int64_t ldx, int64_t N, const double* const* r,
                                   const double* const* B, const int64_t* ldb, const int64_t* n_kept,
                                   const double* const* m_b, const double* const* V_b, const int64_t* ldvb,
                                   const double* logA, const double* lambda0, double* out_host, int* rc_out);

int gpfit_fit_eval_sparse(gpfit_ctx* ctx, void* stream, const double* theta, const double* lower, const double* upper,
                          int n_rows, int n_cols, const double* X, int64_t ldx, int64_t N, const double* Xtilde,
                          int64_t ldxt, int64_t Ntilde, const double* r, const double* B, int64_t ldb, int64_t n_kept,
                          const double* m_b, const double* V_b, int64_t ldvb, double logA, double lambda0,
                          double* out_host);

#define GPFIT_FIT_EVAL_SPARSE_MAX_UNITS 16
int gpfit_fit_eval_sparse_batch(gpfit_ctx* const* ctxs, int n_units, void* stream, const double* theta,
                                const double* lower, const double* upper, int n_rows, int n_cols,
                                const double* const* X, int64_t ldx, int64_t N, const double* const* Xtilde,
                                int64_t ldxt, int64_t Ntilde, const double* const* r, const double* const* B,
                                const int64_t* ldb, const int64_t* n_kept, const double* const* m_b,
                                const double* const* V_b, const int64_t* ldvb, const double* logA,
                                const double* lambda0, double* out_host, int* rc_out);

int gpfit_potrf(gpfit_ctx* ctx, void* stream, const double* A, int64_t lda, int64_t n, double* L, int64_t ldl,
                double* Linv, int64_t ldi, double* logdet_host, int* info_host);

int gpfit_potrf_append(gpfit_ctx* ctx, void* stream, double* L, int64_t ldl, double* Linv, int64_t ldi, int64_t n,
                       const double* kcol, double* logdet_inout_host, int* info_host);

int gpfit_potrf_append_block(gpfit_ctx* ctx, void* stream, double* L, int64_t ldl, double* Linv, int64_t ldi, int64_t n,
                             int64_t k, const double* Kcols, int64_t ldk, double* logdet_inout_host, int* info_host);

int gpfit_estep(gpfit_ctx* ctx, void* stream, const double* K, int64_t ldk, int64_t N, const double* r,
                const double* m, const double* f, double logA, double* m_new, double* V_new, int64_t ldv);

int gpfit_estep_projected(gpfit_ctx* ctx, void* stream, const double* a, int64_t lda, const double* aL, int64_t ldal,
                          const double* L, int64_t ldl, int64_t N, int64_t nb, const double* r, const double* m,
                          const double* f, double logA, double* m_new, double* V_new, int64_t ldv, const double* kv0,
                          double* lam_m_out, double* lam_var_out);

int gpfit_estep_projected_damped(gpfit_ctx* ctx, void* stream, const double* a, int64_t lda, const double* aL,
                                 int64_t ldal, const double* L, int64_t ldl, const double* Linv, int64_t ldli,
                                 const double* V, int64_t ldv_in, int64_t N, int64_t nb, const double* r, const double* m,
                                 const double* f, double logA, double alpha, double* m_new, double* V_new, int64_t ldv,
                                 int* info_v_host);

int gpfit_fparam_eval(gpfit_ctx* ctx, void* stream, const double* lam_m, const double* lam_var,
                      const double* r, int64_t N, double logA, int closed_form_lambda0, double lambda0_in,
                      double* f_out, double* out_host);

int gpfit_fparam_lbfgs(gpfit_ctx* ctx, void* stream, const double* lam_m, const double* lam_var,
                       const double* r, int64_t N, double logA0, int lambda0_mode, double lambda0_fixed,
                       int max_iter, int history_size, double lr, double tol_grad, double tol_change,
                       double* f_out, double* out_host);
int gpfit_fparam_lbfgs_host(const double* lam_m, const double* lam_var, const double* r, int64_t N,
                            double logA0, int lambda0_mode, double lambda0_fixed, int max_iter,
                            int history_size, double lr, double tol_grad, double tol_change, double* f_out,
                            double* out_host);

#define GPFIT_ESTEP_CHAIN_MAX_STEPS 1024
int gpfit_estep_chain(gpfit_ctx* ctx, void* stream, const double* a, int64_t lda, const double* aL, int64_t ldal,
                      const double* L, int64_t ldl, int64_t N, int64_t nb, const double* r, const double* kv0,
                      double* m, double* f, double* V, int64_t ldv, double* lam_m, double* lam_var, double logA0,
                      int lambda0_mode, double lambda0_fixed, int n_steps, int max_iter, int history_size, double lr,
                      double tol_grad, double tol_change, double* rec_host);

int gpfit_estep_chain_full(gpfit_ctx* ctx, void* stream, const double* K, int64_t ldk, int64_t N, const double* r,
                           const double* kv0, double* m, double* f, double* V, int64_t ldv, double* lam_m,
                           double* lam_var, double logA0, int lambda0_mode, double lambda0_fixed, int n_steps,
                           int max_iter, int history_size, double lr, double tol_grad, double tol_change,
                           double* rec_host);

#define GPFIT_ESTEP_CHAIN_MAX_UNITS 16
int gpfit_estep_chain_batch(gpfit_ctx* const* ctxs, int n_units, void* stream, const double* const* a,
                            const int64_t* lda, const double* const* aL, const int64_t* ldal, const double* const* L,
                            const int64_t* ldl, int64_t N, const int64_t* nb, const double* const* r,
                            const double* const* kv0, double* const* m, double* const* f, double* const* V,
                            const int64_t* ldv, double* const* lam_m, double* const* lam_var, const double* logA0,
                            int lambda0_mode, const double* lambda0_fixed, int n_steps, int max_iter, int history_size,
                            double lr, double tol_grad, double tol_change, double* rec_host);

int gpfit_estep_chain_damped(gpfit_ctx* ctx, void* stream, const double* a, int64_t lda, const double* aL, int64_t ldal,
                             const double* L, int64_t ldl, const double* Linv, int64_t ldli, int64_t N, int64_t nb,
                             const double* r, const double* kv0, double* m, double* f, double* V, int64_t ldv,
                             double* lam_m, double* lam_var, double logA0, double alpha, int lambda0_mode,
                             double lambda0_fixed, int n_steps, int max_iter, int history_size, double lr,
                             double tol_grad, double tol_change, double* rec_host);
int gpfit_estep_chain_damped_batch(gpfit_ctx* const* ctxs, int n_units, void* stream, const double* const* a,
                                   const int64_t* lda, const double* const* aL, const int64_t* ldal,
                                   const double* const* L, const int64_t* ldl, const double* const* Linv,
                                   const int64_t* ldli, int64_t N, const int64_t* nb, const double* const* r,
                                   const double* const* kv0, double* const* m, double* const* f, double* const* V,
                                   const int64_t* ldv, double* const* lam_m, double* const* lam_var,
                                   const double* logA0, double alpha, int lambda0_mode, const double* lambda0_fixed,
                                   int n_steps, int max_iter, int history_size, double lr, double tol_grad,
                                   double tol_change, double* rec_host);

#define GPFIT_ESTEP_CHAIN_FULL_MAX_UNITS 16
int gpfit_estep_chain_full_batch(gpfit_ctx* const* ctxs, int n_units, void* stream, const double* const* K,
                                 const int64_t* ldk, int64_t N, const double* const* r, const double* const* kv0,
                                 double* const* m, double* const* f, double* const* V, const int64_t* ldv,
                                 double* const* lam_m, double* const* lam_var, const double* logA0, int lambda0_mode,
                                 const double* lambda0_fixed, int n_steps, int max_iter, int history_size, double lr,
                                 double tol_grad, double tol_change, double* rec_host);

int gpfit_elbo(gpfit_ctx* ctx, void* stream, const double* m, const double* V, int64_t ldv, const double* K, int64_t ldk,
               const double* Kinv, int64_t ldki, int64_t nb, int logdet_K_known, double logdet_K, const double* r,
               const double* f, const double* lam_m, int64_t N, double logA, double lambda0, double* out_host,
               int* info_host);
#define GPFIT_ELBO_MAX_UNITS 16
int gpfit_elbo_batch(gpfit_ctx* const* ctxs, int n_units, void* stream, const double* const* m, const double* const* V,
                     const int64_t* ldv, const double* const* K, const int64_t* ldk, const double* const* Kinv,
                     const int64_t* ldki, const int64_t* nb, const int* logdet_K_known, const double* logdet_K,
                     const double* const* r, const double* const* f, const double* const* lam_m, int64_t N,
                     const double* logA, const double* lambda0, double* out_host, int* info_host);

#define GPFIT_SWEEPS_Y_READY 1
#define GPFIT_SWEEPS_WANT_RR 2
#define GPFIT_SUBSPACE_SWEEPS_MAX_STEPS 1024
int gpfit_subspace_sweeps(gpfit_ctx* ctx, void* stream, const double* K, int64_t ldk, int64_t N, int64_t k, double* Q,
                          double* Y, double* W, double* S, int m, const double* sigma, int flags, int* rec_host);
int gpfit_subspace_sweeps_batch(gpfit_ctx* const* ctxs, int n_units, void* stream, const double* const* K, int64_t ldk,
                                int64_t N, int64_t k, double* const* Q, double* const* Y, double* const* W,
                                double* const* S, const int* m, const double* const* sigma, int flags, int* rec_host);

#define GPFIT_SIGN_CAYLEY 1
#define GPFIT_SIGN_X2_READY 2
#define GPFIT_SIGN_MAX_STEPS 64
int gpfit_sign_steps(gpfit_ctx* ctx, void* stream, const double* S, int64_t k, double tau, double* X, double* X2, double* W,
                     int n_steps, const double* c, int its0, int flags, int* rec_host);
int gpfit_sign_steps_batch(gpfit_ctx* const* ctxs, int n_units, void* stream, const double* const* S, int64_t k,
                           const double* tau, double* const* X, double* const* X2, double* const* W, int n_steps,
                           const double* c, int its0, int flags, int* rec_host);

int gpfit_nd_utility(void* stream, const double* sigma2, const double* mu, int64_t nstar, const double* r,
                     int nr, double* U);

int gpfit_score_pool(gpfit_ctx* ctx, void* stream, double sigma0, const double* xstar, int64_t ldxs, int64_t P,
                     const int* pixels, int64_t d_full, const double* xtilde, int64_t ldxt, int64_t nt, int64_t d,
                     const double* C, int64_t ldc, const double* B, int64_t ldb, int64_t k, const double* S,
                     int64_t lds, const double* w, double A, double lambda0, const double* r, int nr,
                     int64_t chunk_rows, double* mu, double* sigma2, double* rate, double* U);

int gpfit_score_pool_batch(gpfit_ctx* const* ctxs, int n_units, void* stream, const double* sigma0,
                           const double* const* xstar, const int64_t* ldxs, int64_t P, const int* const* pixels,
                           const int64_t* d_full, const double* const* xtilde, const int64_t* ldxt, const int64_t* nt,
                           const int64_t* d, const double* const* C, const int64_t* ldc, const double* const* B,
                           const int64_t* ldb, const int64_t* k, const double* const* S, const int64_t* lds,
                           const double* const* w, const double* A, const double* lambda0, const double* r, int nr,
                           int64_t chunk_rows, double* const* mu, double* const* sigma2, double* const* rate,
                           double* const* U);

int gpfit_utility_sum(void* stream, const double* U, int64_t ldu, int n_rows, const double* weight, int64_t P, double* out);

int gpfit_set_profile(gpfit_ctx* ctx, int on);
int gpfit_get_profile(gpfit_ctx* ctx, double* out16);
int gpfit_get_phases(gpfit_ctx* ctx, double* out8);
double gpfit_last_enqueue_ms(gpfit_ctx* ctx);

int gpfit_fit_eval_f32(gpfit_ctx* ctx, void* stream, const double* theta, const double* lower,
                       const double* upper, int n_rows, int n_cols, const float* X, int64_t ldx, int64_t N,
                       const float* r, const float* m, const float* V, int64_t ldv, double logA, double lambda0,
                       int want_grad, double* out_host, float* lam_m, float* lam_var, float* f);

int gpfit_probe_mfma_f64(void* stream, double* scratch, int blocks, int iters);
int gpfit_probe_stream_copy(void* stream, const double* in, double* out, int64_t n_doubles);

typedef struct gpfit_dev_gemm_args {
  const void* A;
  const void* B;
  void* C;
  int64_t lda, ldb, ldc;
  int64_t sA, sB, sC;
  double alpha, beta;
  void* sk_ws;
  void* aux;
  double* sumsq;
  const void* const* Ap;
  const void* const* Bp;
  void* const* Cp;
  void* const* auxp;
  double* const* sumsqp;
  int32_t M, N, K;
  int32_t a_kmajor, b_kmajor, out_lower, a_tri, b_tri;
  int32_t batch;
  int32_t split_k;
  int32_t tile;
  int32_t walk;
  int32_t epi;
  int32_t nptr;
  int32_t k_slabs;
  int32_t b_split;
} gpfit_dev_gemm_args;

typedef struct gpfit_dev_gemm_route_t {
  int32_t rc;
  int32_t tile;
  int32_t sk_first;
  int32_t xcd;
  int32_t stages;
  int32_t half_occ;
  int32_t edge;
  int32_t epi;
  int32_t sumsq_entries;
  int32_t blocks;
  int32_t pair;
  int32_t slabs;
} gpfit_dev_gemm_route_t;

int gpfit_dev_gemm_route(int is_f32, const gpfit_dev_gemm_args* args, const gpfit_dev_gemm_args* pair_args,
                         gpfit_dev_gemm_route_t* out);
int64_t gpfit_dev_gemm_plan(int is_f32, const gpfit_dev_gemm_args* args, int kind, int32_t* out, int64_t cap);
int gpfit_dev_gemm(void* stream, int is_f32, const gpfit_dev_gemm_args* args, const gpfit_dev_gemm_args* pair_args);
int gpfit_dev_ctx_copy(gpfit_ctx* ctx, const char* name, int64_t offset, void* dev, int64_t bytes, int to_ctx);
int gpfit_dev_ctx_fill(gpfit_ctx* ctx, const char* name, int byte);
int gpfit_dev_potrf(gpfit_ctx* ctx, void* stream, int is_f32, int nb, void* const* A, void* const* L, void* const* Li,
                    void* const* Tmp, int* const* info, int64_t ld, int n, uint32_t need, uint32_t halves, int side_min);

#ifdef __cplusplus
}
#endif
#endif
```

Before: 37.20 fits/s.

## Add grouped GEMM kernel and let off-diagonal products ride along diagonal-block stages

Adds a grouped GEMM launch that runs up to four independent products in one kernel over a host-built, weight-sorted tile table cached on device. In the two-sided top-level update, the independent off-diagonal products (Z21, W21) are sliced and attached to the small recursive diagonal-block GEMMs, which would otherwise leave the GPU underfilled. Whatever remains of those products runs afterwards. The aim is better CU occupancy during small recursive stages, at the cost of a new kernel path, a fixed non-stream-K schedule for the grouped members, and extra host planning on the first call.

Result: no change. 37.30 fits/s, median of 6 (+0.3%).

```diff
diff --git a/gaussian_processes_amd/_lib.py b/gaussian_processes_amd/_lib.py
--- a/gaussian_processes_amd/_lib.py
+++ b/gaussian_processes_amd/_lib.py
@@ -20,7 +20,7 @@
 
 class DevGemmRoute(ctypes.Structure):
     _fields_ = [(n, ctypes.c_int32) for n in ("rc", "tile", "sk_first", "xcd", "stages", "half_occ", "edge", "epi",
-                                              "sumsq_entries", "blocks", "pair", "slabs")]
+                                              "sumsq_entries", "blocks", "pair", "slabs", "group")]
 
 
 _SIGS = {
@@ -100,6 +100,12 @@
     "gpfit_dev_gemm_route": (i32, [i32, ctypes.POINTER(DevGemmArgs), ctypes.POINTER(DevGemmArgs), ctypes.POINTER(DevGemmRoute)]),
     "gpfit_dev_gemm_plan": (i64, [i32, ctypes.POINTER(DevGemmArgs), i32, ctypes.POINTER(ctypes.c_int32), i64]),
     "gpfit_dev_gemm": (i32, [vp, i32, ctypes.POINTER(DevGemmArgs), ctypes.POINTER(DevGemmArgs)]),
+    "gpfit_dev_gemm_group_route": (i32, [i32, i32, ctypes.POINTER(DevGemmArgs), ctypes.POINTER(ctypes.c_int32),
+                                         ctypes.POINTER(ctypes.c_int32), ctypes.POINTER(DevGemmRoute)]),
+    "gpfit_dev_gemm_group_plan": (i64, [i32, i32, ctypes.POINTER(DevGemmArgs), ctypes.POINTER(ctypes.c_int32),
+                                        ctypes.POINTER(ctypes.c_int32), ctypes.POINTER(ctypes.c_int32), i64]),
+    "gpfit_dev_gemm_group": (i32, [vp, i32, i32, ctypes.POINTER(DevGemmArgs), ctypes.POINTER(ctypes.c_int32),
+                                   ctypes.POINTER(ctypes.c_int32)]),
     "gpfit_dev_ctx_copy": (i32, [vp, ctypes.c_char_p, i64, vp, i64, i32]),
     "gpfit_dev_ctx_fill": (i32, [vp, ctypes.c_char_p, i32]),
     "gpfit_dev_potrf": (i32, [vp, vp, i32, i32, vp, vp, vp, vp, vp, i64, i32, ctypes.c_uint32, ctypes.c_uint32, i32]),
diff --git a/gaussian_processes_amd/csrc/api_dev.hip b/gaussian_processes_amd/csrc/api_dev.hip
--- a/gaussian_processes_amd/csrc/api_dev.hip
+++ b/gaussian_processes_amd/csrc/api_dev.hip
@@ -143,6 +143,65 @@
   return d2 ? launch_gemm_pair(a, b, gemm_pair_shape(a, b), s) : launch_gemm(a, s);
 }
 
+template <typename R>
+int group_fill(int n, const gpfit_dev_gemm_args* d, const int32_t* first, const int32_t* count, GemmArgsT<R>* g, GemmSlice* sl) {
+  if (n < 1 || n > GEMM_GROUP_MAX || !d) return -3;
+  for (int i = 0; i < n; ++i) {
+    if (fill(d[i], g[i]) != 0) return -3;
+    sl[i] = {first ? first[i] : 0, count ? count[i] : -1};
+  }
+  return 0;
+}
+template <typename R>
+int group_route(int n, const gpfit_dev_gemm_args* d, const int32_t* first, const int32_t* count, gpfit_dev_gemm_route_t& o) {
+  std::memset(&o, 0, sizeof(o));
+  o.sk_first = -1;
+  GemmArgsT<R> g[GEMM_GROUP_MAX];
+  GemmSlice sl[GEMM_GROUP_MAX];
+  if (group_fill(n, d, first, count, g, sl) != 0) return -3;
+  const GemmRoute h = gemm_group_shape(g, sl, n);
+  o.rc = h.rc; o.tile = h.tile; o.stages = h.stages; o.blocks = h.gx; o.group = h.rc == 0 ? h.tiles : 0;
+  if (h.rc != 0) set_error(h.error);
+  return 0;
+}
+template <typename R>
+int64_t group_plan(int n, const gpfit_dev_gemm_args* d, const int32_t* first, const int32_t* count, int32_t* out, int64_t cap) {
+  GemmArgsT<R> g[GEMM_GROUP_MAX];
+  GemmSlice sl[GEMM_GROUP_MAX];
+  if (group_fill(n, d, first, count, g, sl) != 0) return -3;
+  const GemmRoute h = gemm_group_shape(g, sl, n);
+  if (h.rc != 0) {
+    set_error(h.error);
+    return -1;
+  }
+  GemmGroupShape m[GEMM_GROUP_MAX];
+  for (int i = 0; i < n; ++i) m[i] = {g[i].M, g[i].N, g[i].K, g[i].a_tri, g[i].b_tri, g[i].out_lower, sl[i].first, sl[i].count};
+  std::vector<int> table;
+  if (group_plan_host(m, n, ktile_of<R>(), table) != 0) return -3;
+  const int64_t need = 1 + 5 * (int64_t)table.size();
+  if (need > cap || !out) return need;
+  out[0] = (int32_t)table.size();
+  for (size_t e = 0; e < table.size(); ++e) {
+    const int t = table[e];
+    int32_t* w = out + 1 + 5 * e;
+    if (t < 0) { w[0] = -1; w[1] = w[2] = w[3] = w[4] = 0; continue; }
+    const int mi = t >> 28, ti = (t >> 14) & 0x3fff, tj = t & 0x3fff;
+    const KRange kr = gemm_tile_k_range(m[mi].a_tri, m[mi].b_tri, m[mi].K, ti * TILE, tj * TILE, TILE);
+    w[0] = mi; w[1] = ti; w[2] = tj; w[3] = kr.beg; w[4] = kr.end;
+  }
+  return need;
+}
+template <typename R>
+int group_run(hipStream_t s, int n, const gpfit_dev_gemm_args* d, const int32_t* first, const int32_t* count) {
+  GemmArgsT<R> g[GEMM_GROUP_MAX];
+  GemmSlice sl[GEMM_GROUP_MAX];
+  if (group_fill(n, d, first, count, g, sl) != 0) {
+    set_error("gpfit_dev_gemm_group: 1 to 4 members");
+    return -3;
+  }
+  return launch_gemm_group(g, sl, n, gemm_group_shape(g, sl, n), s);
+}
+
 struct CtxBuf { void* p; int64_t bytes; };
 CtxBuf ctx_buffer(gpfit_ctx* c, const char* name) {
   const int64_t np = c->np_cap, dp = c->dp_cap, nn = np * np * 8;
@@ -196,6 +255,22 @@
                 : gpfit::run<double>((hipStream_t)stream, *args, pair_args);
 }
 
+int gpfit_dev_gemm_group_route(int is_f32, int n, const gpfit_dev_gemm_args* members, const int32_t* first, const int32_t* count,
+                               gpfit_dev_gemm_route_t* out) {
+  if (!out) return -3;
+  return is_f32 ? gpfit::group_route<float>(n, members, first, count, *out) : gpfit::group_route<double>(n, members, first, count, *out);
+}
+
+int64_t gpfit_dev_gemm_group_plan(int is_f32, int n, const gpfit_dev_gemm_args* members, const int32_t* first, const int32_t* count,
+                                  int32_t* out, int64_t cap) {
+  return is_f32 ? gpfit::group_plan<float>(n, members, first, count, out, cap) : gpfit::group_plan<double>(n, members, first, count, out, cap);
+}
+
+int gpfit_dev_gemm_group(void* stream, int is_f32, int n, const gpfit_dev_gemm_args* members, const int32_t* first, const int32_t* count) {
+  return is_f32 ? gpfit::group_run<float>((hipStream_t)stream, n, members, first, count)
+                : gpfit::group_run<double>((hipStream_t)stream, n, members, first, count);
+}
+
 int gpfit_dev_potrf(gpfit_ctx* ctx, void* stream, int is_f32, int nb, void* const* A, void* const* L, void* const* Li,
                     void* const* Tmp, int* const* info, int64_t ld, int n, uint32_t need, uint32_t halves, int side_min) {
   const int64_t elem = is_f32 ? 4 : 8;
diff --git a/gaussian_processes_amd/csrc/common.h b/gaussian_processes_amd/csrc/common.h
--- a/gaussian_processes_amd/csrc/common.h
+++ b/gaussian_processes_amd/csrc/common.h
@@ -3,6 +3,7 @@
 #include <stdint.h>
 #include <stdio.h>
 #include <string>
+#include <vector>
 
 namespace gpfit {
 
@@ -134,6 +135,32 @@
 template <typename R> GemmRoute gemm_pair_shape(const GemmArgsT<R>& a, const GemmArgsT<R>& b);
 template <typename R> int launch_gemm_pair(const GemmArgsT<R>& a, const GemmArgsT<R>& b, const GemmRoute& h, hipStream_t s);
 
+constexpr int GEMM_GROUP_MAX = 4;
+struct GemmSlice { int first, count; };
+template <typename R>
+struct GemmGroupMemberT {
+  const R* A;
+  const R* B;
+  R* C;
+  int64_t lda, ldb, ldc;
+  int M, N, K;
+  double alpha, beta;
+  int a_tri, b_tri, out_lower;
+  int a_kmajor, b_kmajor;
+};
+template <typename R>
+struct GemmGroupArgsT {
+  GemmGroupMemberT<R> m[GEMM_GROUP_MAX];
+  const int* table;
+};
+struct GemmGroupShape { int M, N, K, a_tri, b_tri, out_lower, first, count; };
+int group_member_tiles(const GemmGroupShape& m);
+int group_plan_host(const GemmGroupShape* m, int n, int kt, std::vector<int>& table);
+int group_table_device(const GemmGroupShape* m, int n, int kt, const int** table, int* blocks);
+bool gemm_group_enabled();
+template <typename R> GemmRoute gemm_group_shape(const GemmArgsT<R>* g, const GemmSlice* sl, int n);
+template <typename R> int launch_gemm_group(const GemmArgsT<R>* g, const GemmSlice* sl, int n, const GemmRoute& h, hipStream_t s);
+
 template <typename R>
 struct GramArgsT {
   const R* XCt;
diff --git a/gaussian_processes_amd/csrc/fit.hip b/gaussian_processes_amd/csrc/fit.hip
--- a/gaussian_processes_amd/csrc/fit.hip
+++ b/gaussian_processes_amd/csrc/fit.hip
@@ -205,6 +205,57 @@
   if (e) { e->carried = g.epi != 0; e->sumsq_entries = r.sumsq_entries; }
   return run_gemm(lane.s, g, r);
 }
+template <typename R>
+static int run_gemm_group(hipStream_t s, const GemmArgsT<R>* g, const GemmSlice* sl, int n, const GemmRoute& h) {
+  static int group_no = 0;
+  double flops[GEMM_GROUP_MAX] = {}, total = 0.0;
+  int count[GEMM_GROUP_MAX] = {};
+  if (gemm_logging() || g_prof) {
+    for (int i = 0; i < n; ++i) {
+      const GemmGroupShape m{g[i].M, g[i].N, g[i].K, g[i].a_tri, g[i].b_tri, g[i].out_lower, sl[i].first, sl[i].count};
+      std::vector<int> table;
+      GP_TRY(group_plan_host(&m, 1, ktile_of<R>(), table));
+      for (int e : table) {
+        if (e < 0) continue;
+        const KRange kr = gemm_tile_k_range(m.a_tri, m.b_tri, m.K, ((e >> 14) & 0x3fff) * TILE, (e & 0x3fff) * TILE, TILE);
+        flops[i] += 2.0 * TILE * TILE * std::max(0, kr.end - kr.beg);
+        ++count[i];
+      }
+      total += flops[i];
+    }
+  }
+  if (gemm_logging()) {
+    ++group_no;
+    for (int i = 0; i < n; ++i) {
+      fprintf(stderr, "[gpfit gemm] M %d N %d K %d atri %d btri %d lower %d nb 1 tile %d ak %d bk %d epi 0 flops %.6e", g[i].M, g[i].N,
+              g[i].K, g[i].a_tri, g[i].b_tri, g[i].out_lower, TILE, g[i].a_kmajor, g[i].b_kmajor, flops[i]);
+      gemm_log_tail("", g[i], "");
+      fprintf(stderr, " group %d member %d of %d tiles %d from %d\n", group_no, i, n, count[i], sl[i].first);
+    }
+  }
+  ProfScope ps(s, total, 0);
+  return launch_gemm_group(g, sl, n, h, s);
+}
+
+template <typename R>
+int product_group(Lane lane, const Member<R>* m, int n, bool separate_if_refused) {
+  GemmArgsT<R> g[GEMM_GROUP_MAX];
+  GemmSlice sl[GEMM_GROUP_MAX];
+  bool whole = true;
+  for (int i = 0; i < n && i < GEMM_GROUP_MAX; ++i) {
+    g[i] = product_args(lane, m[i].d, m[i].alpha, m[i].a, m[i].b, m[i].c, m[i].walk);
+    sl[i] = m[i].slice;
+    whole = whole && sl[i].first == 0 && sl[i].count < 0;
+  }
+  const GemmRoute h = gemm_group_shape(g, sl, n);
+  if (h.rc == 0) return run_gemm_group(lane.s, g, sl, n, h);
+  if (!(whole && separate_if_refused)) return 1;
+  for (int i = 0; i < n; ++i) GP_TRY(product(lane, m[i].d, m[i].alpha, m[i].a, m[i].b, m[i].c, m[i].walk));
+  return 0;
+}
+template int product_group<double>(Lane, const Member<double>*, int, bool);
+template int product_group<float>(Lane, const Member<float>*, int, bool);
+
 template int product<double>(Lane, Dims, double, const Operand<double>&, const Operand<double>&, const Output<double>&, int,
                              Epilogue<double>*);
 template int product<float>(Lane, Dims, double, const Operand<float>&, const Operand<float>&, const Output<float>&, int,
@@ -356,17 +407,52 @@
 }
 
 template <typename R>
-static int two_sided_list(Lane lane, int cnt, const TwoSidedBufs<R>* b, const int* r0, int n) {
+struct Rider { Member<R> m; int tiles, next; };
+static int group_round() {
+  static const int v = getenv("GPFIT_GROUP_ROUND") ? atoi(getenv("GPFIT_GROUP_ROUND")) : 1536;
+  return v;
+}
+template <typename R>
+static int ride(Lane lane, Rider<R>& rd, Dims d, double alpha, const Operand<R>& a, const Operand<R>& b, const Output<R>& c, int wk) {
+  const int cnt = c.m.cnt;
+  if (cnt + 1 > GEMM_GROUP_MAX || (d.M % TILE) || (d.N % TILE)) return 1;
+  const int tm = d.M / TILE, own = cnt * (c.lower ? tm * (tm + 1) / 2 : tm * (d.N / TILE));
+  const int slice = std::min(rd.tiles - rd.next, group_round() - own);
+  if (slice <= 0) return 1;
+  Member<R> m[GEMM_GROUP_MAX];
+  for (int i = 0; i < cnt; ++i) {
+    Operand<R> ai = a, bi = b;
+    ai.m.cnt = bi.m.cnt = 1;
+    ai.m.p[0] = a.m.p[i]; bi.m.p[0] = b.m.p[i];
+    Output<R> ci = c;
+    ci.m = mat(c.m.p[i], c.m.ld);
+    m[i] = member(d, alpha, ai, bi, ci, wk);
+  }
+  m[cnt] = sliced(rd.m, rd.next, slice);
+  const int rc = product_group(lane, m, cnt + 1, false);
+  if (rc == 0) rd.next += slice;
+  return rc;
+}
+
+template <typename R>
+static int two_sided_list(Lane lane, int cnt, const TwoSidedBufs<R>* b, const int* r0, int n, Rider<R>* rider = nullptr) {
   if (cnt <= 0) return 0;
   using TS = TwoSidedBufs<R>;
   auto blk = [&](auto X, int dr, int dc) { return ts_blk(cnt, b, r0, X, dr, dc); };
+  auto stage = [&](Lane ln, Dims d, double alpha, const Operand<R>& a_, const Operand<R>& b_, const Output<R>& c_, int wk = 0) -> int {
+    if (rider) {
+      const int rc = ride(ln, *rider, d, alpha, a_, b_, c_, wk);
+      if (rc <= 0) return rc;
+    }
+    return gpfit::product(ln, d, alpha, a_, b_, c_, wk);
+  };
   const int k = n / TILE;
   if (n < b[0].min_split || k < 2) {
     static const int wbase_walk = getenv("GPFIT_WBASE_WALK") ? atoi(getenv("GPFIT_WBASE_WALK")) : 0;
-    GP_TRY(product(lane, {n, n, n}, 1.0, trans(blk(&TS::Q, 0, 0)), plain(tril(blk(&TS::Li, 0, 0))), into(blk(&TS::Z, 0, 0)),
+    GP_TRY(stage(lane, {n, n, n}, 1.0, trans(blk(&TS::Q, 0, 0)), plain(tril(blk(&TS::Li, 0, 0))), into(blk(&TS::Z, 0, 0)),
                    walk(W_RBASE)));
-    return product(lane, {n, n, n}, 0.5, trans(tril(blk(&TS::Li, 0, 0))), plain(blk(&TS::Z, 0, 0)),
-                   into_lower(blk(&TS::W, 0, 0)), wbase_walk);
+    return stage(lane, {n, n, n}, 0.5, trans(tril(blk(&TS::Li, 0, 0))), plain(blk(&TS::Z, 0, 0)),
+                 into_lower(blk(&TS::W, 0, 0)), wbase_walk);
   }
   const int n1 = ((k + 1) / 2) * TILE, n2 = n - n1;
   auto diagonal_blocks = [&]() -> int {
@@ -377,21 +463,21 @@
         bb[2 * i] = b[i]; rr[2 * i] = r0[i];
         bb[2 * i + 1] = b[i]; rr[2 * i + 1] = r0[i] + n1;
       }
-      return two_sided_list<R>(lane, 2 * cnt, bb, rr, n1);
+      return two_sided_list<R>(lane, 2 * cnt, bb, rr, n1, rider);
     }
     for (int i = 0; i < cnt; ++i) rr[i] = r0[i] + n1;
-    GP_TRY(two_sided_list<R>(lane, cnt, b, r0, n1));
-    return two_sided_list<R>(lane, cnt, b, rr, n2);
+    GP_TRY(two_sided_list<R>(lane, cnt, b, r0, n1, rider));
+    return two_sided_list<R>(lane, cnt, b, rr, n2, rider);
   };
-  GP_TRY(product(lane, {n2, n1, n2}, 0.5, trans(blk(&TS::Q, n1, n1)), plain(blk(&TS::Li, n1, 0)), into(blk(&TS::Z, n1, 0))));
+  GP_TRY(stage(lane, {n2, n1, n2}, 0.5, trans(blk(&TS::Q, n1, n1)), plain(blk(&TS::Li, n1, 0)), into(blk(&TS::Z, n1, 0))));
   GP_TRY(dual_update_list(lane, {n2, n1, n1}, 1.0, plain(blk(&TS::Q, n1, 0)), plain(tril(blk(&TS::Li, 0, 0))), blk(&TS::H, n1, 0),
                           blk(&TS::Z, n1, 0), walk(W_H)));
   static const int w21_walk = getenv("GPFIT_W21_WALK") ? atoi(getenv("GPFIT_W21_WALK")) : 0;
-  GP_TRY(product(lane, {n2, n1, n2}, 0.5, trans(tril(blk(&TS::Li, n1, n1))), plain(blk(&TS::Z, n1, 0)),
+  GP_TRY(stage(lane, {n2, n1, n2}, 0.5, trans(tril(blk(&TS::Li, n1, n1))), plain(blk(&TS::Z, n1, 0)),
                  into(blk(&TS::W, n1, 0)), w21_walk));
   GP_TRY(diagonal_blocks());
-  GP_TRY(product(lane, {n1, n1, n2}, 0.5, trans(blk(&TS::Li, n1, 0)), plain(blk(&TS::H, n1, 0)), into_lower(blk(&TS::W, 0, 0), 1.0)));
-  return product(lane, {n1, n1, n2}, 0.5, trans(blk(&TS::H, n1, 0)), plain(blk(&TS::Li, n1, 0)), into_lower(blk(&TS::W, 0, 0), 1.0));
+  GP_TRY(stage(lane, {n1, n1, n2}, 0.5, trans(blk(&TS::Li, n1, 0)), plain(blk(&TS::H, n1, 0)), into_lower(blk(&TS::W, 0, 0), 1.0)));
+  return stage(lane, {n1, n1, n2}, 0.5, trans(blk(&TS::H, n1, 0)), plain(blk(&TS::Li, n1, 0)), into_lower(blk(&TS::W, 0, 0), 1.0));
 }
 
 constexpr int TOP_BLOCKS_MIN = 2048, TOP_BLOCKS_MIN_F32 = 5120;
@@ -407,21 +493,42 @@
   int rr[GEMM_MAXB];
   const int k = n / TILE;
   const int n1 = ((k + 1) / 2) * TILE, n2 = n - n1;
+  static const int w21_walk = getenv("GPFIT_W21_WALK") ? atoi(getenv("GPFIT_W21_WALK")) : 0;
+  static const int group_min = getenv("GPFIT_GROUP_MIN") ? atoi(getenv("GPFIT_GROUP_MIN")) : 4096;
+  static const int group_max = getenv("GPFIT_GROUP_MAX") ? atoi(getenv("GPFIT_GROUP_MAX")) : 4096;
+  Rider<R> z21{member<R>({n2, n1, n2}, 0.5, trans(tril(blk(&TS::Li, n1, n1))), plain(blk(&TS::Q, n1, 0)), into(blk(&TS::Z, n1, 0)), w21_walk),
+               (n2 / TILE) * (n1 / TILE), 0};
+  Rider<R> w21{member<R>({n2, n1, n1}, 1.0, plain(blk(&TS::H, n1, 0)), plain(tril(blk(&TS::Li, 0, 0))), into(blk(&TS::W, n1, 0)), walk(W_H)),
+               (n2 / TILE) * (n1 / TILE), 0};
+  auto rest = [&](Rider<R>& rd) -> int {
+    if (rd.next >= rd.tiles) return 0;
+    if (rd.next == 0) return product(lane, rd.m.d, rd.m.alpha, rd.m.a, rd.m.b, rd.m.c, rd.m.walk);
+    const Member<R> m = sliced(rd.m, rd.next, -1);
+    if (product_group(lane, &m, 1, false) != 0) {
+      set_error("two_sided_top: the rest of a product that rode with the block's stages was refused");
+      return -100;
+    }
+    return 0;
+  };
+  auto admitted = [&](const Rider<R>& rd) {
+    const GemmArgsT<R> g = product_args(lane, rd.m.d, rd.m.alpha, rd.m.a, rd.m.b, rd.m.c, rd.m.walk);
+    const GemmSlice all{0, -1};
+    return gemm_group_shape(&g, &all, 1).rc == 0;
+  };
+  const bool riding = cnt == 1 && sizeof(R) == 8 && n2 >= group_min && n1 <= group_max && admitted(z21) && admitted(w21);
   for (int i = 0; i < cnt; ++i) rr[i] = n1;
-  GP_TRY(two_sided_list<R>(lane, cnt, b, rr, n2));
+  GP_TRY(two_sided_list<R>(lane, cnt, b, rr, n2, riding ? &z21 : nullptr));
   for (int i = 0; i < cnt; ++i) GP_TRY(launch_symmetrize(b[i].W + (int64_t)n1 * ld + n1, ld, n2, s));
-  static const int w21_walk = getenv("GPFIT_W21_WALK") ? atoi(getenv("GPFIT_W21_WALK")) : 0;
-  GP_TRY(product(lane, {n2, n1, n2}, 0.5, trans(tril(blk(&TS::Li, n1, n1))), plain(blk(&TS::Q, n1, 0)),
-                 into(blk(&TS::Z, n1, 0)), w21_walk));
+  GP_TRY(rest(z21));
   GP_TRY(dual_update_list(lane, {n2, n1, n2}, -1.0, plain(blk(&TS::W, n1, n1)), plain(blk(&TS::L, n1, 0)), blk(&TS::H, n1, 0),
                           blk(&TS::Z, n1, 0), 0));
-  GP_TRY(product(lane, {n2, n1, n1}, 1.0, plain(blk(&TS::H, n1, 0)), plain(tril(blk(&TS::Li, 0, 0))), into(blk(&TS::W, n1, 0)),
-                 walk(W_H)));
+  if (!riding) GP_TRY(rest(w21));
   GP_TRY(product(lane, {n1, n1, n2}, -1.0, trans(blk(&TS::L, n1, 0)), plain(blk(&TS::Z, n1, 0)), into_lower(blk(&TS::Q, 0, 0), 1.0)));
   GP_TRY(product(lane, {n1, n1, n2}, -1.0, trans(blk(&TS::Z, n1, 0)), plain(blk(&TS::L, n1, 0)), into_lower(blk(&TS::Q, 0, 0), 1.0)));
   for (int i = 0; i < cnt; ++i) GP_TRY(launch_symmetrize(b[i].Q, ld, n1, s));
   for (int i = 0; i < cnt; ++i) rr[i] = 0;
-  return two_sided_list<R>(lane, cnt, b, rr, n1);
+  GP_TRY(two_sided_list<R>(lane, cnt, b, rr, n1, riding ? &w21 : nullptr));
+  return riding ? rest(w21) : 0;
 }
 
 static double lin_pm1_host(int i, int n) {
diff --git a/gaussian_processes_amd/csrc/gemm.hip b/gaussian_processes_amd/csrc/gemm.hip
--- a/gaussian_processes_amd/csrc/gemm.hip
+++ b/gaussian_processes_amd/csrc/gemm.hip
@@ -7,6 +7,17 @@
 #include <utility>
 
 namespace gpfit {
+
+template <typename R, bool A_KMAJOR, bool B_KMAJOR, bool EDGE, int T, int NS>
+__device__ __forceinline__ void gemm_tile_product(const R* A, int64_t lda, const R* B, int64_t ldb, int M, int N, int row0, int col0,
+                                                  int kbeg, int kend, R* smem, typename Real<R>::acc_t (&acc)[T / 32][T / 32],
+                                                  bool kdesc) {
+#pragma unroll
+  for (int i = 0; i < T / 32; ++i)
+#pragma unroll
+    for (int j = 0; j < T / 32; ++j) acc[i][j] = acc_zero<R>();
+  gemm_mainloop<R, A_KMAJOR, B_KMAJOR, EDGE, T, 0, NS>(A, lda, B, ldb, M, N, row0, col0, kbeg, kend, smem, acc, kdesc);
+}
 
 template <typename R, bool A_KMAJOR, bool B_KMAJOR, bool EDGE, int T, int NS>
 __device__ __forceinline__ bool gemm_tile_compute(const GemmArgsT<R>& p, int tiles_n, int ntiles, R* smem,
@@ -60,14 +71,26 @@
     C += (int64_t)z * p.sC;
   }
 
-#pragma unroll
-  for (int i = 0; i < T / 32; ++i)
-#pragma unroll
-    for (int j = 0; j < T / 32; ++j) acc[i][j] = acc_zero<R>();
-
-  gemm_mainloop<R, A_KMAJOR, B_KMAJOR, EDGE, T, 0, NS>(A, p.lda, B, p.ldb, p.M, p.N, row0, col0, kbeg, kend, smem, acc,
-                                                       (p.reverse & 4) != 0);
+  gemm_tile_product<R, A_KMAJOR, B_KMAJOR, EDGE, T, NS>(A, p.lda, B, p.ldb, p.M, p.N, row0, col0, kbeg, kend, smem, acc,
+                                                        (p.reverse & 4) != 0);
   return true;
+}
+
+template <typename R, bool EDGE, int T>
+__device__ __forceinline__ void gemm_tile_store(const typename Real<R>::acc_t (&acc)[T / 32][T / 32], int row0, int col0,
+                                                R* C, int64_t ldc, int M, int N, R alpha, R beta) {
+  if (beta == (R)0) {
+    for_each_acc<R, T>(acc, row0, col0, [&](int row, int col, R v) {
+      if (!EDGE || (row < M && col < N)) C[(int64_t)row * ldc + col] = alpha * v;
+    });
+  } else {
+    for_each_acc<R, T>(acc, row0, col0, [&](int row, int col, R v) {
+      if (!EDGE || (row < M && col < N)) {
+        R* c = C + (int64_t)row * ldc + col;
+        *c = alpha * v + beta * (*c);
+      }
+    });
+  }
 }
 
 template <typename R, bool A_KMAJOR, bool B_KMAJOR, bool EDGE, int T, int NS, int EPI = 0>
@@ -119,18 +142,7 @@
     }
     return;
   }
-  if (beta == (R)0) {
-    for_each_acc<R, T>(acc, row0, col0, [&](int row, int col, R v) {
-      if (!EDGE || (row < M && col < N)) C[(int64_t)row * ldc + col] = alpha * v;
-    });
-  } else {
-    for_each_acc<R, T>(acc, row0, col0, [&](int row, int col, R v) {
-      if (!EDGE || (row < M && col < N)) {
-        R* c = C + (int64_t)row * ldc + col;
-        *c = alpha * v + beta * (*c);
-      }
-    });
-  }
+  gemm_tile_store<R, EDGE, T>(acc, row0, col0, C, ldc, M, N, alpha, beta);
 }
 
 template <typename R, bool A_KMAJOR, bool B_KMAJOR, bool EDGE, int T, int NS = 2>
@@ -451,6 +463,97 @@
 template int launch_gemm_pair<double>(const GemmArgsT<double>&, const GemmArgsT<double>&, const GemmRoute&, hipStream_t);
 template int launch_gemm_pair<float>(const GemmArgsT<float>&, const GemmArgsT<float>&, const GemmRoute&, hipStream_t);
 
+template <typename R, bool A_KMAJOR>
+__device__ __forceinline__ void gemm_group_tile(const GemmGroupMemberT<R>& m, int ti, int tj, R* smem) {
+  typename Real<R>::acc_t acc[TILE / 32][TILE / 32];
+  const int row0 = ti * TILE, col0 = tj * TILE;
+  const KRange kr = gemm_tile_k_range(m.a_tri, m.b_tri, m.K, row0, col0, TILE);
+  gemm_tile_product<R, A_KMAJOR, true, false, TILE, 2>(m.A, m.lda, m.B, m.ldb, m.M, m.N, row0, col0, kr.beg, kr.end, smem, acc, false);
+  gemm_tile_store<R, false, TILE>(acc, row0, col0, m.C, m.ldc, m.M, m.N, (R)m.alpha, (R)m.beta);
+}
+
+template <typename R>
+__global__ __launch_bounds__(GEMM_THREADS, 2) void gemm_group_kernel(GemmGroupArgsT<R> q) {
+  __shared__ __attribute__((aligned(16))) R smem[4 * Real<R>::KT * TILE];
+  const int e = __builtin_amdgcn_readfirstlane(q.table[blockIdx.x]);
+  if (e < 0) return;
+  const GemmGroupMemberT<R>& m = q.m[(e >> 28) & (GEMM_GROUP_MAX - 1)];
+  const int ti = (e >> 14) & 0x3fff, tj = e & 0x3fff;
+  if (m.a_kmajor) gemm_group_tile<R, true>(m, ti, tj, smem);
+  else gemm_group_tile<R, false>(m, ti, tj, smem);
+}
+
+bool gemm_group_enabled() {
+  static const bool on = !(getenv("GPFIT_GROUP") && atoi(getenv("GPFIT_GROUP")) == 0);
+  return on;
+}
+
+template <typename R>
+GemmRoute gemm_group_shape(const GemmArgsT<R>* g, const GemmSlice* sl, int n) {
+  GemmRoute h{};
+  h.sk_first = -1;
+  auto refuse = [&](const char* why) {
+    h.rc = -3;
+    h.error = why;
+    return h;
+  };
+  if (!gemm_group_enabled()) return refuse("launch_gemm_group: group launches are switched off (GPFIT_GROUP=0)");
+  if (n < 1 || n > GEMM_GROUP_MAX) return refuse("launch_gemm_group: a group holds 1 to 4 members");
+  long tiles = 0;
+  for (int i = 0; i < n; ++i) {
+    const GemmArgsT<R>& a = g[i];
+    if (a.M <= 0 || a.N <= 0 || (a.M % TILE) || (a.N % TILE) || a.M / TILE >= (1 << 14) || a.N / TILE >= (1 << 14))
+      return refuse("launch_gemm_group: a member needs whole 128-tiles");
+    if (a.nptr > 0 || a.batch > 1) return refuse("launch_gemm_group: a member is one problem, not a batch");
+    if (a.epi) return refuse("launch_gemm_group: a member cannot carry a fused epilogue");
+    if (a.split_k > 1 || a.k_slabs > 0 || a.b_split != 0) return refuse("launch_gemm_group: no split-k, k_slabs or split op(B) in a group");
+    if (a.half_occ || (a.reverse & 4)) return refuse("launch_gemm_group: no half-occupancy member and none that walks k downwards");
+    if (!a.b_kmajor) return refuse("launch_gemm_group: no instance for this layout pair (op(B) must be k-major)");
+    const GemmRoute own = gemm_route(a);
+    if (own.rc != 0) return refuse(own.error);
+    if (own.sched == GEMM_STREAMK) return refuse("launch_gemm_group: the member's own route is stream-K (its bits would change)");
+    const GemmGroupShape m{a.M, a.N, a.K, a.a_tri, a.b_tri, a.out_lower, sl[i].first, sl[i].count};
+    const int all = group_member_tiles(m), cnt = sl[i].count < 0 ? all - sl[i].first : sl[i].count;
+    if (sl[i].first < 0 || cnt <= 0 || sl[i].first + cnt > all) return refuse("launch_gemm_group: a slice must be a non-empty range of the member's tiles");
+    tiles += cnt;
+  }
+  h.tile = TILE;
+  h.tiles = (int)tiles;
+  h.stages = 2;
+  h.gx = (int)round_up(tiles, 8);
+  h.gy = h.gz = 1;
+  return h;
+}
+template GemmRoute gemm_group_shape<double>(const GemmArgsT<double>*, const GemmSlice*, int);
+template GemmRoute gemm_group_shape<float>(const GemmArgsT<float>*, const GemmSlice*, int);
+
+template <typename R>
+int launch_gemm_group(const GemmArgsT<R>* g, const GemmSlice* sl, int n, const GemmRoute& h, hipStream_t s) {
+  if (h.rc != 0) {
+    set_error(h.error);
+    return h.rc;
+  }
+  static_assert(sizeof(GemmGroupArgsT<R>) <= 4096, "kernel arguments are limited to 4 KiB");
+  GemmGroupArgsT<R> q{};
+  GemmGroupShape shapes[GEMM_GROUP_MAX];
+  for (int i = 0; i < n; ++i) {
+    const GemmArgsT<R>& a = g[i];
+    q.m[i] = {a.A, a.B, a.C, a.lda, a.ldb, a.ldc, a.M, a.N, a.K, a.alpha, a.beta, a.a_tri, a.b_tri, a.out_lower, a.a_kmajor, a.b_kmajor};
+    shapes[i] = {a.M, a.N, a.K, a.a_tri, a.b_tri, a.out_lower, sl[i].first, sl[i].count};
+  }
+  int blocks = 0;
+  GP_TRY(group_table_device(shapes, n, ktile_of<R>(), &q.table, &blocks));
+  if (blocks != h.gx) {
+    set_error("launch_gemm_group: the table does not have the route's length");
+    return -100;
+  }
+  hipLaunchKernelGGL((gemm_group_kernel<R>), dim3(blocks), dim3(GEMM_THREADS), 0, s, q);
+  GP_HIP(hipGetLastError());
+  return 0;
+}
+template int launch_gemm_group<double>(const GemmArgsT<double>*, const GemmSlice*, int, const GemmRoute&, hipStream_t);
+template int launch_gemm_group<float>(const GemmArgsT<float>*, const GemmSlice*, int, const GemmRoute&, hipStream_t);
+
 template int launch_gemm<double>(const GemmArgsT<double>&, const GemmRoute&, hipStream_t);
 template int launch_gemm<float>(const GemmArgsT<float>&, const GemmRoute&, hipStream_t);
 template int launch_gemm_plain<double>(const GemmArgsT<double>&, const GemmRoute&, hipStream_t);
diff --git a/gaussian_processes_amd/csrc/gemm_sched.hip b/gaussian_processes_amd/csrc/gemm_sched.hip
--- a/gaussian_processes_amd/csrc/gemm_sched.hip
+++ b/gaussian_processes_amd/csrc/gemm_sched.hip
@@ -126,4 +126,67 @@
 template int launch_gemm_xcd<double>(const GemmArgsT<double>&, GemmRoute, hipStream_t);
 template int launch_gemm_xcd<float>(const GemmArgsT<float>&, GemmRoute, hipStream_t);
 
+int group_member_tiles(const GemmGroupShape& m) {
+  const int tm = m.M / TILE, tn = m.N / TILE;
+  return m.out_lower ? tm * (tm + 1) / 2 : tm * tn;
 }
+
+namespace {
+struct GroupTile { int weight, entry; };
+void group_member_walk(const GemmGroupShape& m, int member, int kt, std::vector<GroupTile>& out) {
+  const int tm = m.M / TILE, tn = m.N / TILE;
+  for (int ti = 0; ti < tm; ++ti)
+    for (int tj = 0; tj < (m.out_lower ? ti + 1 : tn); ++tj) {
+      const KRange kr = gemm_tile_k_range(m.a_tri, m.b_tri, m.K, ti * TILE, tj * TILE, TILE);
+      out.push_back({std::max(0, kr.end - kr.beg) / kt, (member << 28) | (ti << 14) | tj});
+    }
+  std::stable_sort(out.begin(), out.end(), [](const GroupTile& x, const GroupTile& y) { return x.weight > y.weight; });
+}
+}
+
+int group_plan_host(const GemmGroupShape* m, int n, int kt, std::vector<int>& table) {
+  table.clear();
+  if (n < 1 || n > GEMM_GROUP_MAX) return -3;
+  std::vector<GroupTile> all;
+  for (int i = 0; i < n; ++i) {
+    if (m[i].M <= 0 || m[i].N <= 0 || (m[i].M % TILE) || (m[i].N % TILE) || m[i].M / TILE >= (1 << 14) ||
+        m[i].N / TILE >= (1 << 14) || (m[i].out_lower && m[i].M != m[i].N))
+      return -3;
+    std::vector<GroupTile> own;
+    group_member_walk(m[i], i, kt, own);
+    const int cnt = m[i].count < 0 ? (int)own.size() - m[i].first : m[i].count;
+    if (m[i].first < 0 || cnt < 0 || m[i].first + cnt > (int)own.size()) return -3;
+    all.insert(all.end(), own.begin() + m[i].first, own.begin() + m[i].first + cnt);
+  }
+  std::stable_sort(all.begin(), all.end(), [](const GroupTile& x, const GroupTile& y) { return x.weight > y.weight; });
+  table.assign((size_t)round_up((int64_t)all.size(), 8), -1);
+  for (size_t e = 0; e < all.size(); ++e) table[e] = all[e].entry;
+  return 0;
+}
+
+int group_table_device(const GemmGroupShape* m, int n, int kt, const int** table, int* blocks) {
+  static std::map<std::vector<int>, Plan> plans;
+  int device = 0;
+  GP_HIP(hipGetDevice(&device));
+  std::vector<int> key{device, kt, n};
+  for (int i = 0; i < n; ++i) key.insert(key.end(), {m[i].M, m[i].N, m[i].K, m[i].a_tri, m[i].b_tri, m[i].out_lower, m[i].first, m[i].count});
+  std::lock_guard<std::mutex> lock(g_mutex);
+  auto it = plans.find(key);
+  if (it == plans.end()) {
+    std::vector<int> host;
+    if (group_plan_host(m, n, kt, host) != 0 || host.empty()) {
+      set_error("launch_gemm_group: the members have no tile table (gemm_group_shape says so beforehand)");
+      return -3;
+    }
+    Plan np;
+    np.blocks = (int)host.size();
+    GP_HIP(hipMalloc((void**)&np.table, host.size() * sizeof(int)));
+    GP_HIP(hipMemcpy(np.table, host.data(), host.size() * sizeof(int), hipMemcpyHostToDevice));
+    it = plans.emplace(key, np).first;
+  }
+  *table = it->second.table;
+  *blocks = it->second.blocks;
+  return 0;
+}
+
+}
diff --git a/gaussian_processes_amd/csrc/product.h b/gaussian_processes_amd/csrc/product.h
--- a/gaussian_processes_amd/csrc/product.h
+++ b/gaussian_processes_amd/csrc/product.h
@@ -1,5 +1,6 @@
 #pragma once
 #include "context.h"
+#include <initializer_list>
 #include <type_traits>
 
 namespace gpfit {
@@ -82,4 +83,15 @@
 int product(Lane lane, Dims d, double alpha, const Operand<R>& a, const Operand<R>& b, const Output<R>& c, int walk = 0,
             Epilogue<R>* e = nullptr);
 
+template <typename R> struct Member { Dims d; double alpha; Operand<R> a, b; Output<R> c; int walk; GemmSlice slice; };
+template <typename R>
+Member<R> member(Dims d, double alpha, const Operand<R>& a, const Operand<R>& b, const Output<R>& c, int walk = 0) {
+  return {d, alpha, a, b, c, walk, {0, -1}};
 }
+template <typename R> Member<R> sliced(Member<R> m, int first, int count) { m.slice = {first, count}; return m; }
+template <typename R> int product_group(Lane lane, const Member<R>* m, int n, bool separate_if_refused = true);
+template <typename R> int product_group(Lane lane, std::initializer_list<Member<R>> m, bool separate_if_refused = true) {
+  return product_group(lane, m.begin(), (int)m.size(), separate_if_refused);
+}
+
+}
diff --git a/include/gpfit_mi355x.h b/include/gpfit_mi355x.h
--- a/include/gpfit_mi355x.h
+++ b/include/gpfit_mi355x.h
@@ -278,12 +278,18 @@
   int32_t blocks;
   int32_t pair;
   int32_t slabs;
+  int32_t group;
 } gpfit_dev_gemm_route_t;
 
 int gpfit_dev_gemm_route(int is_f32, const gpfit_dev_gemm_args* args, const gpfit_dev_gemm_args* pair_args,
                          gpfit_dev_gemm_route_t* out);
 int64_t gpfit_dev_gemm_plan(int is_f32, const gpfit_dev_gemm_args* args, int kind, int32_t* out, int64_t cap);
 int gpfit_dev_gemm(void* stream, int is_f32, const gpfit_dev_gemm_args* args, const gpfit_dev_gemm_args* pair_args);
+int gpfit_dev_gemm_group_route(int is_f32, int n, const gpfit_dev_gemm_args* members, const int32_t* first, const int32_t* count,
+                               gpfit_dev_gemm_route_t* out);
+int64_t gpfit_dev_gemm_group_plan(int is_f32, int n, const gpfit_dev_gemm_args* members, const int32_t* first, const int32_t* count,
+                                  int32_t* out, int64_t cap);
+int gpfit_dev_gemm_group(void* stream, int is_f32, int n, const gpfit_dev_gemm_args* members, const int32_t* first, const int32_t* count);
 int gpfit_dev_ctx_copy(gpfit_ctx* ctx, const char* name, int64_t offset, void* dev, int64_t bytes, int to_ctx);
 int gpfit_dev_ctx_fill(gpfit_ctx* ctx, const char* name, int byte);
 int gpfit_dev_potrf(gpfit_ctx* ctx, void* stream, int is_f32, int nb, void* const* A, void* const* L, void* const* Li,
```
